# fverdoja/Fast-3D-Pointcloud-Segmentation

Hardware: AMD Instinct MI355X
Metric: Mpoints/sec segmented end-to-end, 1M-pt RGB-D frames (higher is better)
Workload: dtype f32

## Files before the change

### fast-3d-pointcloud-segmentation_amd/csrc/f3ds_algo.h

```cpp
#ifndef F3DS_ALGO_H_
#define F3DS_ALGO_H_

#include "f3ds_numerics.h"

namespace f3ds {

#define F3DS_MAX_SEED_EVENTS 48
struct SeedEvent {
    int trigger;
    int depth;
    double min[3];
    unsigned off[3];
};
struct SeedGrid {
    int n_events;
    int error;
    int defined;
    int depth;
    double res;
    double min[3], max[3];
    unsigned off[3];
    SeedEvent ev[F3DS_MAX_SEED_EVENTS];
};
F3DS_HD void a_seed_init(SeedGrid& g, float seed_res) {
// ... 398 lines not shown
    }
    *owner_out = o; *dist_out = d;
}
F3DS_HD void a_centroid_finish(const float sum[9], unsigned count, float row[12]) {
    float nx = sum[6], ny = sum[7], nz = sum[8];
    float z = (nx * nx + ny * ny) + (nz * nz + 0.0f);
    if (z > 0.0f) { float q = n_sqrtf(z); nx /= q; ny /= q; nz /= q; }
    float c = (float)count;
    row[0] = sum[0] / c; row[1] = sum[1] / c; row[2] = sum[2] / c;
    row[3] = sum[3] / c; row[4] = sum[4] / c; row[5] = sum[5] / c;
    row[6] = nx; row[7] = ny; row[8] = nz;
    row[9] = row[10] = row[11] = 0.0f;
}

F3DS_HD void a_payload_row(const float* vf_row, float out[12]) {
    float x = vf_row[0], y = vf_row[1], z = vf_row[2];
    out[0] = x * x; out[1] = x * y; out[2] = x * z; out[3] = y * y; out[4] = y * z; out[5] = z * z;
    out[6] = x; out[7] = y; out[8] = z;
    out[9] = (float)((uint32_t)vf_row[3] & 255u);
    out[10] = (float)((uint32_t)vf_row[4] & 255u);
    out[11] = (float)((uint32_t)vf_row[5] & 255u);
}
F3DS_HD void a_fold_row(float acc[12], const float row[12], unsigned index_plus_1) {
    for (int k = 0; k < 9; ++k) acc[k] += row[k];
    float count = (float)index_plus_1;
    float inv = 1 / count;
    for (int k = 9; k < 12; ++k) acc[k] = acc[k] + inv * (row[k] - acc[k]);
}
F3DS_HD void a_region_from_acc(const float acc[12], unsigned count, float rec[16]) {
    float c = (float)count;
    rec[0] = acc[6] / c; rec[1] = acc[7] / c; rec[2] = acc[8] / c;
    float n4[4];
    n_plane_normal(acc, count, rec, n4);
    rec[3] = n4[0]; rec[4] = n4[1]; rec[5] = n4[2];
    rec[6] = acc[9]; rec[7] = acc[10]; rec[8] = acc[11];
    n_rgb2lab(rec + 6, rec + 9);
    rec[12] = rec[13] = rec[14] = rec[15] = 0.0f;
}

struct MergeParams {
    int color_metric, geom_metric, merging;
    float lambda;
    int bins;
    const float* cdf_c;
    const float* cdf_g;
};
F3DS_HD float a_tc(const MergeParams& p, float dc, int* err) {
    if (p.merging != 2) return p.lambda * dc;
    short bin = (short)__builtin_floorf(dc * (float)(short)p.bins);
    if (bin == (short)p.bins) bin--;
    if (bin < 0 || bin >= (short)p.bins) { *err = -9; return 0.0f; }
    return p.cdf_c[bin] / 2;
}
F3DS_HD float a_tg(const MergeParams& p, float dg, int* err) {
    if (p.merging != 2) return (1 - p.lambda) * dg;
    short bin = (short)__builtin_floorf(dg * (float)(short)p.bins);
    if (bin < 0 || bin >= (short)p.bins) { *err = -9; return 0.0f; }
    return p.cdf_g[bin] / 2;
}
template <class K = m_lit> F3DS_HD float a_edge_weight(const MergeParams& p, const float* rec_first, const float* rec_second, int* err, K mc = K()) {
    float dc, dg;
    n_delta_c_g(rec_first, rec_second, p.color_metric, p.geom_metric, &dc, &dg, mc);
    return a_tc(p, dc, err) + a_tg(p, dg, err);
}

struct EdgeHist {
    const uint32_t* ev_epoch;
    const uint32_t* ev_key;
    const int* ev_prev;
};
F3DS_HD bool a_edge_before(const EdgeHist& H, uint32_t e, uint32_t ke, int he, uint32_t f, uint32_t kf, int hf) {
    if (ke != kf) return ke < kf;
    for (;;) {
        uint32_t te = H.ev_epoch[he], tf = H.ev_epoch[hf];
        uint32_t tau = te > tf ? te : tf;
        if (tau == 0u) return e < f;
        if (te == tau) he = H.ev_prev[he];
        if (tf == tau) hf = H.ev_prev[hf];
        ke = H.ev_key[he]; kf = H.ev_key[hf];
        if (ke != kf) return ke < kf;
    }
}

}
#endif
```

### fast-3d-pointcloud-segmentation_amd/csrc/f3ds_hip.hip

```cpp
#include <hip/hip_runtime.h>

#include <algorithm>
#include <cmath>
#include <atomic>
#include <map>
#include <chrono>
#include <cstdio>
#include <cstdlib>
#include <cstring>
#include <string>
#include <type_traits>
#include <mutex>
#include <set>
#include <vector>

#include "../../include/f3ds.h"
#include "f3ds_algo.h"
#include "f3ds_glasbey.h"
#include "f3ds_eval.h"
#include "f3ds_dev.h"
#include "f3ds_levels.h"

using namespace f3ds;

#include "f3ds_kernels.inc"
#include "f3ds_levels.inc"

namespace {

thread_local std::string g_last_hip_error;
#define HIPCHECK(expr) do { hipError_t e_ = (expr); if (e_ != hipSuccess) { g_last_hip_error = std::string(#expr) + ": " + hipGetErrorString(e_); return F3DS_ERR_HIP; } } while (0)

template <class... Ts> struct ArgPack;
template <> struct ArgPack<> {};
template <class T, class... Ts> struct ArgPack<T, Ts...> { T head; ArgPack<Ts...> tail; };

template <class K, class... Done>
__device__ __forceinline__ void unpack_call(const ArgPack<>&, Done... d) { K{}(d...); }
template <class K, class T, class... Ts, class... Done>
__device__ __forceinline__ void unpack_call(const ArgPack<T, Ts...>& p, Done... d) { unpack_call<K>(p.tail, d..., p.head); }

template <class K, class = void> struct waves_per_simd { static constexpr int v = 1; };
template <class K> struct waves_per_simd<K, std::void_t<decltype(K::WAVES_PER_SIMD)>> { static constexpr int v = K::WAVES_PER_SIMD; };
template <class K, class = void> struct is_latency_kernel { static constexpr bool v = false; };
template <class K> struct is_latency_kernel<K, std::void_t<decltype(K::LATENCY_KERNEL)>> { static constexpr bool v = K::LATENCY_KERNEL; };
template <class K, class Pack>
__global__ __launch_bounds__(K::BLOCK, waves_per_simd<K>::v) void k_batched(const Pack* frames) {
#ifndef F3DS_EXP_NO_LATENCY_PRIO
    if constexpr (is_latency_kernel<K>::v) __builtin_amdgcn_s_setprio(3);
#endif
    const Pack p = frames[f3ds_frame()];
    unpack_call<K>(p);
}

template <class F> struct op_traits;
template <class C, class... Ps> struct op_traits<void (C::*)(Ps...) const> { using pack = ArgPack<std::decay_t<Ps>...>; };
template <class K> using pack_of = typename op_traits<decltype(&K::operator())>::pack;

inline void fill_pack(ArgPack<>&) {}
template <class T, class... Ts, class A, class... As>
inline void fill_pack(ArgPack<T, Ts...>& p, A a, As... as) {
    static_assert(std::is_convertible<A, T>::value && !(std::is_pointer<T>::value && std::is_integral<A>::value),
                  "rec<K>(): an argument does not convert implicitly to the kernel's parameter type (wrong element type, swapped arguments?)");
    p.head = a; fill_pack(p.tail, as...);
}

typedef hipError_t (*LaunchFn)(uint32_t gx, uint32_t nf, uint32_t lds, hipStream_t st, const void* dargs);
template <class K>
hipError_t launch_fn(uint32_t gx, uint32_t nf, uint32_t lds, hipStream_t st, const void* dargs) {
    using Pack = pack_of<K>;
    if (lds > 48u * 1024u) {
        hipError_t e = hipFuncSetAttribute(reinterpret_cast<const void*>(k_batched<K, Pack>), hipFuncAttributeMaxDynamicSharedMemorySize, (int)lds);
        if (e != hipSuccess) return e;
    }
    hipLaunchKernelGGL((k_batched<K, Pack>), dim3(gx ? gx : 1u, nf), dim3(K::BLOCK), lds, st, static_cast<const Pack*>(dargs));
    return hipGetLastError();
}
struct Cmd { LaunchFn fn; uint32_t gx, lds, bytes, off; };

const int g_inc_shift = [] { const char* e = dev_getenv("F3DS_INC_SHIFT"); return e ? atoi(e) : 6; }();

struct Switches {
    bool direct_labels = false, copy_stream = true, copy_duplex = false, split_voxel_accum = false, sweep_tiles = true, merge_spec = true, force_global_merge = false, no_stream_pool = false, sort_pairs = false, host_prof = false, trace_err = false, vox_hash = true, vox_tiles_forced = false, levels_global = false;
    int normals_threads = 0, merge_nw = 0, merge_keys = -1; uint32_t tile_holes = 0, ilist_slack = 32, r_rounds = F3DS_R_ROUNDS; long relabel_lds_cap = -1;
    void read() {
        auto on = [](const char* n) { return dev_getenv(n) != nullptr; };
        auto num = [](const char* n, long dflt) { const char* e = dev_getenv(n); return e ? atol(e) : dflt; };
        direct_labels = num("F3DS_DIRECT_LABELS", 0) != 0; copy_stream = num("F3DS_COPY_STREAM", 1) != 0; copy_duplex = num("F3DS_COPY_STREAM", 1) == 2; split_voxel_accum = on("F3DS_SPLIT_VOXEL_ACCUM"); sweep_tiles = num("F3DS_SWEEP_TILES", 1) != 0; merge_spec = num("F3DS_MERGE_SPEC", 1) != 0;
        force_global_merge = on("F3DS_FORCE_GLOBAL_MERGE"); no_stream_pool = on("F3DS_NO_STREAM_POOL"); sort_pairs = on("F3DS_SORT_PAIRS");
        host_prof = on("F3DS_HOST_PROF"); trace_err = on("F3DS_TRACE_ERR");
        vox_tiles_forced = num("F3DS_VOX_TILES", 1) == 2;
        vox_hash = num("F3DS_VOX_TILES", 1) != 0 && !sort_pairs && !split_voxel_accum;
        normals_threads = (int)num("F3DS_NORMALS_THREADS", 0); tile_holes = (uint32_t)num("F3DS_SWEEP_TILE_HOLES", 0);
        { const long v = num("F3DS_MERGE_NW", 0); merge_nw = v == 4 ? 4 : (v ? 8 : 0); }
        { const char* e = dev_getenv("F3DS_MERGE_KEYS"); merge_keys = !e ? -1 : (!strcmp(e, "lds") ? 2 : (!strcmp(e, "global") ? 1 : 0)); }
        relabel_lds_cap = num("F3DS_RELABEL_LDS_CAP", -1);
        levels_global = num("F3DS_LEVELS_GLOBAL", 0) != 0;
        { const long v = num("F3DS_R_ROUNDS_RUN", F3DS_R_ROUNDS); r_rounds = v >= 1 && v <= F3DS_R_ROUNDS ? (uint32_t)v : (uint32_t)F3DS_R_ROUNDS; }
        { const long v = num("F3DS_ILIST_SLACK", 32); ilist_slack = v >= 1 && v <= 32 ? (uint32_t)v : 32u; }
    }
};
thread_local Switches g_sw;
const int g_merge_shared_res = [] { const char* e = dev_getenv("F3DS_MERGE_SHARED_RES"); return e && atoi(e) == 2 ? 2 : 0; }();

#define F3DS_SCRATCH(X) \
    X(P16, pts) X(P16, spts) X(uint64_t, keys0) X(uint64_t, keys1) X(uint32_t, vals0) X(uint32_t, vals1) X(uint32_t, flags) X(uint32_t, incl) X(uint32_t, tiles) X(uint32_t, hist) X(uint32_t, seg_start) X(int, pt_voxel) X(uint32_t, labels) \
    X(uint32_t, vkey) X(uint32_t, vcount) X(float, vf) X(int, nbr) X(int, nbrT) X(uint64_t, hkeys) X(uint32_t, hvals) X(float, boxes) X(uint32_t, ckey) X(uint32_t, cell_start) X(uint64_t, chk) X(uint32_t, chv) X(uint32_t, chvals) X(int, seed_orig) X(uint32_t, keep) X(int, seed_kept) \
    X(uint32_t, owner0) X(uint32_t, ownR) X(float, dist0) X(unsigned char, R) X(float, hc) X(uint32_t, hcount) X(uint32_t, hlo) X(uint32_t, hhi) X(int, ghost_vox) X(unsigned char, ghost_active) X(unsigned char, ghost_done) X(uint32_t, ghost_head) X(uint32_t, ghost_next) \
    X(uint32_t, loff) X(float, rows) X(int, row_voxel) X(float, racc0) X(uint32_t, rcnt0) X(float, rrec0) X(unsigned char, ralive0) X(uint64_t, ehk) X(uint64_t, ekeys0) X(uint64_t, ekeys1) X(uint32_t, evals0) X(uint32_t, evals1) X(uint32_t, ea0) X(uint32_t, eb0) \
    X(uint32_t, ea) X(uint32_t, eb) X(float, ew) X(uint32_t, eku) X(int, ehist) X(unsigned char, ealive) X(uint32_t, ev_epoch) X(uint32_t, ev_key) X(int, ev_prev) X(float, racc) X(uint32_t, rcnt) X(float, rrec) X(unsigned char, ralive) X(uint32_t, rhead) X(uint32_t, rtail) X(uint32_t, lnext) X(uint32_t, parent) X(uint32_t, markA) X(uint32_t, markB) X(uint32_t, tl) X(uint32_t, merges) \
     X(float, r_vf) X(uint32_t, r_owner) X(float, r_dist) X(float, r_hc) X(uint32_t, r_hcount) X(uint32_t, r_hlo) X(uint32_t, r_hhi) X(int, r_gvox) X(unsigned char, r_gact) X(unsigned char, r_gdone) X(uint32_t, r_ghead) X(uint32_t, r_gnext) X(uint32_t, r_tl) X(uint32_t, r_tcnt) X(int, r_seed) X(uint32_t, r_L) \
    X(uint32_t, tstamp) X(uint32_t, tround) X(uint32_t, hdirty) X(uint32_t, htiles) X(uint32_t, htcnt) X(uint32_t, vwl) X(uint32_t, vwl2) X(uint32_t, vtmask) \
     X(uint32_t, glut) X(uint32_t, truth_pts) X(uint32_t, tsum) X(uint32_t, tcol) X(uint32_t, tlab) X(uint32_t, ctab) X(uint32_t, csize) X(uint32_t, eroot) X(uint32_t, eincl) \
     X(uint32_t, hcnt) X(uint32_t, pslot) X(uint32_t, vlist) \
     X(uint32_t, u_src) X(uint32_t, u_voff) X(float, u_xyz) X(uint32_t, u_rgba) X(float, u_cent) X(float, u_nrm) \
    X(float, deltas) X(uint64_t, skeys0) X(uint64_t, skeys1) X(uint32_t, svals0) X(uint32_t, svals1) X(uint32_t, cdf_hist) X(float, cdf) X(uint32_t, root) X(uint32_t, rincl) X(uint32_t, rrank) X(uint2, pool) X(uint32_t, rstart) X(uint32_t, rnleaf) X(uint32_t, rcap) X(uint32_t, tile_n1) X(uint32_t, tile_ord) X(uint32_t, tile_slots) X(uint32_t, ilist) X(uint32_t, istart) X(uint32_t, ilen) X(uint32_t, icap) \
     X(uint32_t, lv_into) X(uint32_t, lv_at) X(uint32_t, lv_pfx) X(float, lv_thr) X(uint32_t, lv_tab) X(uint32_t, lv_nreg) X(uint32_t, lv_out)
template <class T> struct Scratch { T* p = nullptr; size_t cap = 0; int slot = -1; };
#define F3DS_SCRATCH_SLOT(T, name) S_##name,
#define F3DS_SCRATCH_MEMBER(T, name) Scratch<T> name{nullptr, 0, S_##name};
#define F3DS_SCRATCH_VISIT(T, name) if (const int rc_ = f(name)) return rc_;
enum ScratchSlot { F3DS_SCRATCH(F3DS_SCRATCH_SLOT) N_SCRATCH };

}

struct f3ds_ctx {
    int device = 0;
    hipStream_t own_stream = nullptr;
    hipStream_t stream = nullptr;
    hipEvent_t ev[11] = {};
    DevCounters* d_dc = nullptr;
    DevCounters* h_dc = nullptr;
    GridInfo* d_grid = nullptr;
    GridInfo* h_grid = nullptr;
    SeedGrid* d_sgrid = nullptr;
    std::vector<Cmd> cmds;
    std::vector<unsigned char> blob;
    std::vector<uintptr_t> pend;
    MultiOp ops = {}; uint32_t ops_grid = 0;
    unsigned char* h_args[2] = {nullptr, nullptr}; unsigned char* d_args[2] = {nullptr, nullptr}; size_t args_cap = 0;
    hipEvent_t ev_args[2] = {nullptr, nullptr}; bool args_used[2] = {false, false}; int args_flip = 0;
    hipEvent_t ev_copy[3] = {nullptr, nullptr, nullptr};
    DevCounters* d_dcblk = nullptr; DevCounters* h_dcblk = nullptr; size_t dcblk_cap = 0;
    bool have_frame = false;
    bool live = false;
    int rc = 0;
    f3ds_params prm;
    FrameArgs fa;
    const P16* d_pts = nullptr;
    uint32_t n = 0, V = 0, C = 0, S0 = 0, E = 0, hmask = 0;
    uint64_t *ks = nullptr; uint32_t *vs = nullptr;
    uint64_t *cks = nullptr; uint32_t *cvs = nullptr;
    uint64_t *eks = nullptr;
    f3ds_result res;
    bool merge_in_lds = false;
    int merge_kind = 0;
    uint32_t ev_mult = 64;
    uint32_t pool_mult = 1;
    uint32_t vox_cap = 0;
    bool vox_hashed = false;
    bool vox_dense = false;
    uint32_t vox_dense_wait = 0, vox_dense_penalty = 8;
    uint32_t ilist_mult = 1;
    uint32_t edge_mult = 32;
    bool relabel_lds = true;
    int refined_itr = -1;
    int idxbits = -1;
    uint32_t* user_labels = nullptr;
    MergeDev mdev; MergeLds mlds; float host_lambda = 0.5f;
    F3DS_SCRATCH(F3DS_SCRATCH_MEMBER)
    template <class F> int each_scratch(F&& f) { F3DS_SCRATCH(F3DS_SCRATCH_VISIT) return 0; }
    std::vector<uint32_t> tsize;
    float cluster_T = 0.0f;
    bool user_mode = false;
    std::vector<uint32_t> user_label, user_row;
};

namespace {

bool referenced_by_pending_calls(const f3ds_ctx* c, const void* mem, size_t cap) {
    const uintptr_t lo = (uintptr_t)mem, hi = lo + cap;
    for (const uintptr_t w : c->pend) if (w >= lo && w < hi) return true;
    for (uint32_t k = 0; k < c->ops.n; ++k) {
        const uintptr_t d = (uintptr_t)c->ops.dst[k], sp = (uintptr_t)c->ops.src[k];
        if ((d >= lo && d < hi) || (sp >= lo && sp < hi)) return true;
    }
    return false;
}
template <class A> inline void note_arg(f3ds_ctx* c, const A& a) {
    if constexpr (std::is_pointer<A>::value) { if (a) c->pend.push_back((uintptr_t)a); }
    else if constexpr (std::is_class<A>::value) {
        static_assert(std::is_trivially_copyable<A>::value, "kernel arguments must be plain data");
        for (size_t off = 0; off + 8 <= sizeof(A); off += 8) { uintptr_t w; memcpy(&w, reinterpret_cast<const unsigned char*>(&a) + off, 8); if (w) c->pend.push_back(w); }
    }
}
std::atomic<size_t> g_scratch_hwm[16][N_SCRATCH];
std::atomic<unsigned long long> g_scratch_allocs{0};
template <class T>
int regrow(Scratch<T>& b, size_t mark) {
    g_scratch_allocs.fetch_add(1, std::memory_order_relaxed);
    if (b.p) { HIPCHECK(hipFree(b.p)); b.p = nullptr; b.cap = 0; }
    const size_t want = mark + mark / 4 + 64;
    HIPCHECK(hipMalloc(&b.p, want));
    b.cap = want;
    return F3DS_OK;
}
template <class T>
int ensure(f3ds_ctx* c, Scratch<T>& b, size_t count, T** out) {
    size_t bytes = count * sizeof(T);
    if (bytes < 256) bytes = 256;
    size_t target = bytes;
    std::atomic<size_t>& hwm = g_scratch_hwm[c->device & 15][b.slot];
    size_t seen = hwm.load(std::memory_order_relaxed);
    while (seen < bytes && !hwm.compare_exchange_weak(seen, bytes, std::memory_order_relaxed)) {}
    if (seen > target && seen <= 4 * bytes) target = seen;
    if (b.cap < bytes) {
        if (b.p && (!c->cmds.empty() || c->ops.n) && referenced_by_pending_calls(c, b.p, b.cap)) {
            fprintf(stderr, "f3ds: internal error: regrowing a buffer that a recorded kernel call refers to\n");
            return F3DS_ERR_LOGIC;
        }
        static const bool trace = dev_getenv("F3DS_TRACE_ALLOC") != nullptr;
        if (trace && b.p) fprintf(stderr, "f3ds: regrow slot %d: cap %zu, request %zu, mark %zu, pending calls %zu\n", b.slot, b.cap, bytes, target, c->cmds.size());
        if (const int rc = regrow(b, target)) return rc;
    }
    *out = b.p;
    return F3DS_OK;
}
int pregrow_scratch(f3ds_ctx* c) {
    return c->each_scratch([c](auto& b) -> int {
        if (!b.p) return F3DS_OK;
        const size_t mark = g_scratch_hwm[c->device & 15][b.slot].load(std::memory_order_relaxed);
        if (b.cap >= mark || mark > 4 * b.cap) return F3DS_OK;
        return regrow(b, mark);
    });
}
#define ENSURE(buf, count, ptr) do { int rc_ = ensure(c, buf, (size_t)(count), &ptr); if (rc_) return rc_; } while (0)

thread_local size_t g_grid_cap = 2048;
thread_local int g_batch_frames = 1;
std::atomic<int> g_batch_calls[16];
struct BatchCallCount { int d; explicit BatchCallCount(int dev) : d(dev & 15) { g_batch_calls[d].fetch_add(1, std::memory_order_relaxed); } ~BatchCallCount() { g_batch_calls[d].fetch_sub(1, std::memory_order_relaxed); } };
size_t grid_cap_for_batch(int frames) {
    static const size_t target = dev_getenv("F3DS_GRID_TARGET") ? (size_t)atol(dev_getenv("F3DS_GRID_TARGET")) : 3072;
    if (!target) return 2048;
    size_t cap = target / (size_t)(frames > 0 ? frames : 1);
    return cap < 8 ? 8 : (cap > 2048 ? 2048 : cap);
}
inline uint32_t grid_wide(size_t work, int block) {
    size_t g = (work + block - 1) / block;
    return (uint32_t)(g < 1 ? 1 : (g > 2048 ? 2048 : g));
}
inline uint32_t grid_for(size_t work, int block) {
    size_t g = (work + block - 1) / block;
    if (g < 1) g = 1;
    if (g > g_grid_cap) g = g_grid_cap;
    return (uint32_t)g;
}
inline uint32_t pow2_ge(size_t x) { uint32_t p = 1; while (p < x) p <<= 1; return p; }
int bits_for(uint64_t max_value) { int b = 0; while (b < 64 && (max_value >> b)) ++b; return b; }

template <class K, class... As> void rec(f3ds_ctx* c, uint32_t gx, uint32_t lds, As... as);
inline void flush_ops(f3ds_ctx* c) {
    if (!c->ops.n) return;
    const MultiOp m = c->ops; const uint32_t g = c->ops_grid;
    c->ops.n = 0; c->ops_grid = 0;
    rec<d_multi_op>(c, g, 0u, m);
}
template <class K, class... As>
void rec(f3ds_ctx* c, uint32_t gx, uint32_t lds, As... as) {
    if constexpr (!std::is_same<K, d_multi_op>::value) flush_ops(c);
    using Pack = pack_of<K>;
    static_assert(std::is_trivially_copyable<Pack>::value, "kernel arguments must be plain data");
    Pack p;
    memset(&p, 0, sizeof p);
    fill_pack(p, as...);
    (note_arg(c, as), ...);
    Cmd cmd; cmd.fn = &launch_fn<K>; cmd.gx = gx; cmd.lds = lds; cmd.bytes = (uint32_t)sizeof(Pack); cmd.off = (uint32_t)c->blob.size();
    c->blob.resize(c->blob.size() + sizeof(Pack));
    memcpy(c->blob.data() + cmd.off, &p, sizeof(Pack));
    c->cmds.push_back(cmd);
}
inline void rec_op(f3ds_ctx* c, void* dst, const void* src, uint32_t value, size_t bytes) {
    const uint32_t words = (uint32_t)((bytes + 3) / 4);
    if (c->ops.n == (uint32_t)MULTI_OPS) flush_ops(c);
    MultiOp& m = c->ops;
    if (m.n == 0) memset(&m, 0, sizeof m);
    m.dst[m.n] = static_cast<uint32_t*>(dst); m.src[m.n] = static_cast<const uint32_t*>(src); m.val[m.n] = value; m.words[m.n] = words; m.n++;
    const uint32_t g = grid_for(words, 256);
    if (g > c->ops_grid) c->ops_grid = g;
}
inline void rec_fill(f3ds_ctx* c, void* dst, uint32_t value, size_t bytes) { rec_op(c, dst, nullptr, value, bytes); }
inline void rec_copy(f3ds_ctx* c, void* dst, const void* src, size_t bytes) { rec_op(c, dst, src, 0u, bytes); }
inline void reset_recording(f3ds_ctx* c) { c->cmds.clear(); c->blob.clear(); c->pend.clear(); c->ops.n = 0; c->ops_grid = 0; }

struct Batch {
    std::vector<f3ds_ctx*> fr;
    hipStream_t st = nullptr;
    f3ds_ctx* owner = nullptr;
};

thread_local double g_t_wait = 0, g_t_launch = 0;
static int trace_err(int code, const char* where, const f3ds_ctx* c) {
    if (code && g_sw.trace_err)
        fprintf(stderr, "f3ds: error %d after %s (V %u, seeds %u, edges %u, chain overflow %d, capacity flag %d)\n", code, where, c->V, c->S0, c->h_dc->n_edges,
                c->h_dc->r_overflow, c->h_dc->ev_overflow);
    return code;
}
static inline double now_ms() { return std::chrono::duration<double, std::milli>(std::chrono::steady_clock::now().time_since_epoch()).count(); }
inline hipError_t timed_sync(hipEvent_t e) { const double t0 = now_ms(); const hipError_t r = hipEventSynchronize(e); g_t_wait += now_ms() - t0; return r; }
inline hipError_t timed_sync(hipStream_t st) { const double t0 = now_ms(); const hipError_t r = hipStreamSynchronize(st); g_t_wait += now_ms() - t0; return r; }
template <class F> int clear_counter(f3ds_ctx* c, hipStream_t st, F DevCounters::*f) { c->h_dc->*f = 0; HIPCHECK(hipMemsetAsync(&(c->d_dc->*f), 0, sizeof(F), st)); return F3DS_OK; }
template <class... Fs> int clear_counters(f3ds_ctx* c, hipStream_t st, Fs DevCounters::*... f) { int rc = F3DS_OK; (void)((rc = clear_counter(c, st, f)) || ...); return rc; }
int flush(Batch& b, hipEvent_t before_launch = nullptr) {
    if (b.fr.empty()) return F3DS_OK;
    for (f3ds_ctx* c : b.fr) flush_ops(c);
    const size_t ncmd = b.fr[0]->cmds.size();
    for (f3ds_ctx* c : b.fr) if (c->cmds.size() != ncmd) return F3DS_ERR_UNSUPPORTED;
    if (ncmd == 0) return F3DS_OK;
    const uint32_t nf = (uint32_t)b.fr.size();
    size_t total = 0;
    std::vector<size_t> off(ncmd);
    for (size_t j = 0; j < ncmd; ++j) { off[j] = total; total += (((size_t)b.fr[0]->cmds[j].bytes * nf) + 63u) & ~(size_t)63u; }
    f3ds_ctx* o = b.owner;
    if (o->args_cap < total) {
        HIPCHECK(hipStreamSynchronize(b.st));
        for (int k = 0; k < 2; ++k) {
            if (o->h_args[k]) HIPCHECK(hipHostFree(o->h_args[k]));
            if (o->d_args[k]) HIPCHECK(hipFree(o->d_args[k]));
            o->h_args[k] = o->d_args[k] = nullptr; o->args_used[k] = false;
        }
        o->args_cap = total * 2;
        for (int k = 0; k < 2; ++k) {
            HIPCHECK(hipHostMalloc(&o->h_args[k], o->args_cap, hipHostMallocDefault));
            HIPCHECK(hipMalloc(&o->d_args[k], o->args_cap));
            if (!o->ev_args[k]) HIPCHECK(hipEventCreateWithFlags(&o->ev_args[k], hipEventDisableTiming));
        }
    }
    const int fl = o->args_flip; o->args_flip ^= 1;
    if (o->args_used[fl]) HIPCHECK(timed_sync(o->ev_args[fl]));
    unsigned char* const h_args = o->h_args[fl]; unsigned char* const d_args = o->d_args[fl];
    const double tl0 = now_ms();
    for (size_t j = 0; j < ncmd; ++j)
        for (uint32_t i = 0; i < nf; ++i) {
            const Cmd& cm = b.fr[i]->cmds[j];
            if (cm.fn != b.fr[0]->cmds[j].fn) return F3DS_ERR_UNSUPPORTED;
            memcpy(h_args + off[j] + (size_t)i * cm.bytes, b.fr[i]->blob.data() + cm.off, cm.bytes);
        }
    HIPCHECK(hipMemcpyAsync(d_args, h_args, total, hipMemcpyHostToDevice, b.st));
    if (before_launch) HIPCHECK(hipEventRecord(before_launch, b.st));
    for (size_t j = 0; j < ncmd; ++j) {
        uint32_t gx = 1, lds = 0;
        for (uint32_t i = 0; i < nf; ++i) { const Cmd& cm = b.fr[i]->cmds[j]; if (cm.gx > gx) gx = cm.gx; if (cm.lds > lds) lds = cm.lds; }
        HIPCHECK(b.fr[0]->cmds[j].fn(gx, nf, lds, b.st, d_args + off[j]));
    }
    HIPCHECK(hipEventRecord(o->ev_args[fl], b.st)); o->args_used[fl] = true;
    for (f3ds_ctx* c : b.fr) reset_recording(c);
    g_t_launch += now_ms() - tl0;
    return F3DS_OK;
}
int flush_sync(Batch& b) {
    int rc = flush(b);
    if (rc) return rc;
    const size_t nf = b.fr.size();
    if (nf == 1) HIPCHECK(hipMemcpyAsync(b.fr[0]->h_dc, b.fr[0]->d_dc, sizeof(DevCounters), hipMemcpyDeviceToHost, b.st));
    else if (nf > 1) {
        f3ds_ctx* o = b.owner;
        if (o->dcblk_cap < nf) {
            HIPCHECK(hipStreamSynchronize(b.st));
            if (o->d_dcblk) HIPCHECK(hipFree(o->d_dcblk));
            if (o->h_dcblk) HIPCHECK(hipHostFree(o->h_dcblk));
            o->dcblk_cap = nf * 2;
            HIPCHECK(hipMalloc(&o->d_dcblk, o->dcblk_cap * sizeof(DevCounters)));
            HIPCHECK(hipHostMalloc(&o->h_dcblk, o->dcblk_cap * sizeof(DevCounters), hipHostMallocDefault));
        }
        for (size_t i = 0; i < nf; ++i) rec<d_dc_gather>(b.fr[i], 1u, 0u, b.fr[i]->d_dc, o->d_dcblk + i);
        if ((rc = flush(b))) return rc;
        HIPCHECK(hipMemcpyAsync(o->h_dcblk, o->d_dcblk, nf * sizeof(DevCounters), hipMemcpyDeviceToHost, b.st));
    }
    HIPCHECK(timed_sync(b.st));
    HIPCHECK(hipGetLastError());
    if (nf > 1) for (size_t i = 0; i < nf; ++i) *b.fr[i]->h_dc = b.owner->h_dcblk[i];
// ... 207 lines not shown
    if (sb.reseed) {
        rec<d_reseed_own>(c, grid_for(S0, 256), 0u, sb.seeds, S0, owner0);
        rec<d_reseed_init>(c, grid_for(S0 + 1, 256), 0u, sb.seeds, S0, owner0, ghost_vox, ghost_active, ghost_done, hlo, hhi, hcount, tl, tcnt);
    } else {
        rec<d_helper_own>(c, grid_for(S0, 256), 0u, sb.seeds, S0, owner0);
        rec<d_helper_init>(c, grid_for(S0 + 1, 256), 0u, sb.seeds, S0, owner0, ghost_vox, ghost_active, ghost_done, hlo, hhi, hcount, hc, tl, tcnt);
    }
    const int* nbrT = c->nbrT.p; const float* vf = sb.vf;
    SweepFrame a;
    a.sv = SweepView{(int)V, nbrT, vf, owner0, dist0, hc, ghost_head, ghost_next, &c->d_dc->n_ghosts, prm.seed_res, prm.w_normal, prm.w_color, prm.w_spatial, c->nbr.p};
    a.R = R; a.ownR = ownR; a.owner_out = owner0; a.dist_out = dist0;
    a.ghost_done = ghost_done; a.ghost_active = ghost_active; a.ghost_vox = ghost_vox; a.ghost_head = ghost_head; a.ghost_next = ghost_next;
    a.hlo = hlo; a.hhi = hhi; a.hcount = hcount; a.hc = hc; a.dc = c->d_dc; a.S0 = S0;
    a.tR0 = tiles4; a.tR1 = tiles4 + T; a.tC0 = tiles4 + 2 * (size_t)T; a.tC1 = tiles4 + 3 * (size_t)T; a.tRr = trr; a.hD = hD; a.T = T; a.tl = tl; a.tcnt = tcnt; a.wl = wl; a.wl2 = wl2; a.tmask = tmask;
    a.thr = g_inc_shift >= 32 ? 0xFFFFFFFFu : (g_inc_shift < 0 ? 0u : V >> g_inc_shift);
    if (!g_sw.sweep_tiles) a.tile_n1 = nullptr;
    else a.tile_n1 = c->tile_n1.p;
    a.tile_ord = c->tile_ord.p; a.tile_slots = c->tile_slots.p;
    for (uint32_t t = 0; t < c->res.sweeps; ++t) {
        if (a_sweep_needs_clear(t)) rec_fill(c, R, 0u, V);
        rec<d_sweep_begin>(c, 1u, 0u, a, t);
        const bool can_skip = t >= 2u;
        const bool rounds = g_inc_shift >= 0 && can_skip;
        const uint32_t nrounds = rounds ? g_sw.r_rounds : 0u;
        rec<d_sweep_R_first>(c, grid_for(V, 256), 0u, a, a_sweep_tag(t), t, nrounds);
        for (uint32_t r = 1; r < nrounds; ++r) rec<d_sweep_R_round>(c, grid_for(V, 256), 0u, a, t, r, nrounds);
        for (uint32_t pass = 0; pass < F3DS_R_PASSES; ++pass) rec<d_sweep_R>(c, pass == 0 ? grid_for(V, 256) : 64u, 0u, a, a_sweep_tag(t), t, pass);
        rec<d_sweep_R_tail>(c, 1u, 0u, a, a_sweep_tag(t), t);
        rec<d_sweep_claim>(c, grid_for(V, 256), 0u, a, t);
        rec<d_centroid>(c, grid_for((size_t)S0 * 64u, 256), 0u, a, t);
    }
    return F3DS_OK;
}
int seg_sweeps(f3ds_ctx* c) {
    SweepBufs sb{&c->owner0, &c->dist0, &c->hc, &c->hcount, &c->hlo, &c->hhi, &c->ghost_vox, &c->ghost_active, &c->ghost_done, &c->ghost_head, &c->ghost_next, &c->htiles, &c->htcnt, c->vf.p, c->seed_kept.p, false};
    return seg_sweeps_on(c, sb);
}
int seg_supervoxels(f3ds_ctx* c) {
    const uint32_t V = c->V, S0 = c->S0;
    uint32_t *loff, *rcnt0, *ev0, *ev1; float *rows, *racc0, *rrec0; int* row_voxel; unsigned char* ralive0; uint64_t *ehk, *ek0, *ek1;
    ENSURE(c->loff, S0 + 2, loff);
    int rc = scan_u32(c, c->hcount.p, loff + 1, S0 + 1);
    if (rc) return rc;
    rec_fill(c, loff, 0u, 4);
    ENSURE(c->rows, ((size_t)V + S0 + 1) * 12, rows); ENSURE(c->row_voxel, (size_t)V + S0 + 1, row_voxel);
    ENSURE(c->racc0, (size_t)(S0 + 1) * 12, racc0); ENSURE(c->rcnt0, S0 + 1, rcnt0); ENSURE(c->rrec0, (size_t)(S0 + 1) * 16, rrec0);
    ENSURE(c->ralive0, S0 + 1, ralive0);
    rec_fill(c, ralive0, 0u, S0 + 1);
    rec_fill(c, rcnt0, 0u, (size_t)(S0 + 1) * 4);
    rec<d_sv_fill>(c, S0 ? (S0 + 3u) / 4u : 1u, 0u,
                   c->vf.p, c->owner0.p, S0, c->hlo.p, c->hhi.p, c->ghost_vox.p, c->ghost_active.p, c->hcount.p, loff, c->hc.p, rows, row_voxel, racc0, rcnt0, rrec0, ralive0, c->d_dc, c->htiles.p, c->htcnt.p, V);
    const uint32_t ecap = (uint32_t)std::min<uint64_t>((uint64_t)S0 * c->edge_mult + 1024u, 0x7fffffffu);
    const uint32_t ehcap = pow2_ge((size_t)ecap * 2);
    ENSURE(c->ehk, ehcap, ehk);
    ENSURE(c->ekeys0, ecap, ek0); ENSURE(c->ekeys1, ecap, ek1); ENSURE(c->evals0, ecap, ev0); ENSURE(c->evals1, ecap, ev1);
    rec_fill(c, ehk, 0xFFFFFFFFu, (size_t)ehcap * 8);
    rec<d_edges>(c, grid_for(V, 256), 0u, V, S0, c->nbrT.p, c->owner0.p, ehk, ehcap - 1, ek0, ecap, c->d_dc);
    rec<d_edges_ghost>(c, grid_for(S0, 256), 0u, V, S0, c->ghost_vox.p, c->ghost_active.p, c->nbrT.p, c->owner0.p, ehk, ehcap - 1, ek0, ecap, c->d_dc);
    return F3DS_OK;
}
int seg_edge_sort(f3ds_ctx* c, int sort_bits) {
    const uint32_t E = c->E, S0 = c->S0;
    uint32_t *ea0, *eb0; ENSURE(c->ea0, E, ea0); ENSURE(c->eb0, E, eb0);
    uint32_t* evs;
    { uint32_t* h; ENSURE(c->hist, (size_t)RS_BINS * (((size_t)E * 2 + RS_TILE - 1) / RS_TILE + 1), h); }
    rec<d_iota>(c, grid_for(E, 256), 0u, c->evals0.p, E);
    int rc = radix_sort(c, c->ekeys0.p, c->evals0.p, c->ekeys1.p, c->evals1.p, E, sort_bits, &c->eks, &evs);
    if (rc) return rc;
    rec<d_edge_init>(c, grid_for(E, 256), 0u, c->eks, E, S0, ea0, eb0);
    return F3DS_OK;
}
bool merge_il_layout(uint32_t E, uint32_t S0, int nw, int res, MergeLds* xl) {
    memset(xl, 0, sizeof *xl);
    if ((uint64_t)E * (res == 2 ? 10u : 2u) > (1u << 22)) return false;
    const MergeIlLayout L = merge_il_offsets(E, nw, res);
    xl->Ecap = L.Ecap; xl->NGcap = L.NGcap; xl->lds_bytes = L.total; xl->keys_in_lds = res;
    xl->spec = g_sw.merge_spec ? 1 : 0;
    return L.total <= MC_LDS_LIMIT && S0 <= 65534u;
}
enum MergeKind { MK_GLOBAL = 0, MK_IL = 1 };
inline int mk_waves(int kind) { return (kind - MK_IL) >= 2 ? 4 : 8; }
inline int mk_res(int kind) { return (kind - MK_IL) % 2 ? 0 : 2; }
int choose_merge_kind(const std::vector<f3ds_ctx*>& fr, bool force_global) {
    if (force_global || g_sw.force_global_merge) return MK_GLOBAL;
    const bool e_keys = g_sw.merge_keys >= 0;
    const bool shared = fr.size() >= 16 && g_batch_calls[fr[0]->device & 15].load(std::memory_order_relaxed) >= 2;
    const int nw = g_sw.merge_nw ? (g_sw.merge_nw == 8 ? 8 : 4) : (shared ? 4 : 8);
    const int first = e_keys ? (g_sw.merge_keys == 2 ? 2 : 0) : (shared ? g_merge_shared_res : 2);
    for (int res = first; res >= (e_keys ? first : 0); res -= 2) {
        bool ok = true;
        for (f3ds_ctx* c : fr) { MergeLds t; if (!merge_il_layout(c->E, c->S0, nw, res, &t)) { ok = false; break; } }
        if (ok) return MK_IL + (nw == 8 ? 0 : 2) + (res == 2 ? 0 : 1);
    }
    return MK_GLOBAL;
}
int seg_cluster_front(f3ds_ctx* c, const f3ds_params* prm, int kind) {
    const bool use_lds = kind != MK_GLOBAL;
    const uint32_t S0 = c->S0, E = c->E;
    float lambda = 0.5f; int bins = 500;
    if (prm->merging == F3DS_MANUAL_LAMBDA && prm->lambda != 0) { if (prm->lambda < 0 || prm->lambda > 1) return F3DS_ERR_RANGE; lambda = prm->lambda; }
    if (prm->merging == F3DS_EQUALIZATION && prm->bins != 0) { if (prm->bins < 0) return F3DS_ERR_RANGE; bins = (short)prm->bins; }
    if (prm->merging < 0 || prm->merging > 2 || prm->color_metric < 0 || prm->color_metric > 1 || prm->geom_metric < 0 || prm->geom_metric > 1) return F3DS_ERR_ARG;
    MergeDev m;
    memset(&m, 0, sizeof m);
    m.E = E; m.S0 = S0; m.threshold = prm->threshold; m.dc = c->d_dc;
    { const uint64_t cap = (uint64_t)E * c->ev_mult + 4096u; m.ev_cap = cap > 0x7fffffffull ? 0x7fffffffu : (uint32_t)cap; }
    ENSURE(c->ea, E, m.ea); ENSURE(c->eb, E, m.eb); ENSURE(c->ew, ((size_t)E + 2047) & ~(size_t)2047, m.ew);  ENSURE(c->eku, ((size_t)E + 2047) & ~(size_t)2047, m.eku);
    ENSURE(c->ehist, E, m.ehist); ENSURE(c->ealive, E, m.ealive);
    ENSURE(c->ev_epoch, m.ev_cap, m.ev_epoch); ENSURE(c->ev_key, m.ev_cap, m.ev_key); ENSURE(c->ev_prev, m.ev_cap, m.ev_prev);
    ENSURE(c->racc, (size_t)(S0 + 1) * 12, m.racc); ENSURE(c->rrec, (size_t)(S0 + 1) * 16, m.rrec);
    ENSURE(c->rcnt, S0 + 1, m.rcnt); ENSURE(c->ralive, S0 + 1, m.ralive);
    ENSURE(c->rhead, S0 + 1, m.rhead); ENSURE(c->rtail, S0 + 1, m.rtail); ENSURE(c->lnext, S0 + 1, m.lnext);
    ENSURE(c->parent, S0 + 1, m.parent); ENSURE(c->markA, S0 + 1, m.markA); ENSURE(c->markB, S0 + 1, m.markB);
    ENSURE(c->tl, E, m.tl); ENSURE(c->merges, (size_t)(S0 + 1) * 3, m.merges);
    m.loff = c->loff.p; m.llen = c->hcount.p; m.rows = c->rows.p;
    float* deltas; ENSURE(c->deltas, (size_t)E * 2, deltas);
    rec_copy(c, m.racc, c->racc0.p, (size_t)(S0 + 1) * 12 * 4);
    rec_copy(c, m.rrec, c->rrec0.p, (size_t)(S0 + 1) * 16 * 4);
    rec_copy(c, m.rcnt, c->rcnt0.p, (size_t)(S0 + 1) * 4);
    rec_copy(c, m.ralive, c->ralive0.p, (size_t)(S0 + 1));
    rec_copy(c, m.ea, c->ea0.p, (size_t)E * 4);
    rec_copy(c, m.eb, c->eb0.p, (size_t)E * 4);
    MergeLds xl;
    merge_il_layout(E, S0, use_lds ? mk_waves(kind) : 8, use_lds ? mk_res(kind) : 0, &xl);
    uint32_t logS = 1; while ((1u << logS) < S0 + 2u) ++logS;
    xl.pool_cap = (S0 + 1u) * (4u * logS + 8u) * c->pool_mult;
    ENSURE(c->pool, xl.pool_cap, xl.pool); ENSURE(c->rstart, S0 + 1, xl.rstart); ENSURE(c->rnleaf, S0 + 1, xl.rnleaf);
    ENSURE(c->rcap, S0 + 1, xl.rcap);
    if (use_lds) {
        const uint64_t bound = 2ull * E + (uint64_t)(S0 ? S0 - 1u : 0u) * (MC_TL_CAP + MC_TL_CAP / 2u + 4u) + 1024u;
        uint64_t cap = 2ull * E + (uint64_t)g_sw.ilist_slack * E * c->ilist_mult + (g_sw.ilist_slack < 32u ? 16u : 1024u);
        if (cap > bound) cap = bound;
        xl.ilist_cap = cap > 0x7fffffffull ? 0x7fffffffu : (uint32_t)cap;
        ENSURE(c->ilist, xl.ilist_cap, xl.ilist); ENSURE(c->istart, S0 + 1, xl.istart); ENSURE(c->ilen, S0 + 1, xl.ilen); ENSURE(c->icap, S0 + 1, xl.icap);
    }
    if (use_lds) rec<d_inc_build>(c, 1u, 0u, E, S0, m.ea, m.eb, xl.istart, xl.ilen, xl.icap, xl.ilist);
    xl.stop_key = (prm->threshold != prm->threshold) ? 0u : n_weight_key(prm->threshold);
    c->merge_in_lds = use_lds; c->merge_kind = kind;
    rec<d_region_reset>(c, grid_for(S0 + 1, 256), 0u, S0, c->hcount.p, m.rhead, m.rtail, m.lnext, m.parent, m.markA, m.markB, xl.pool, xl.rstart, xl.rnleaf, xl.rcap, c->loff.p);
    m.mp.color_metric = prm->color_metric; m.mp.geom_metric = prm->geom_metric; m.mp.merging = prm->merging; m.mp.lambda = lambda; m.mp.bins = bins;
    uint64_t *sk0 = nullptr, *sk1 = nullptr; uint32_t *sv0 = nullptr, *sv1 = nullptr;
    if (prm->merging == F3DS_ADAPTIVE_LAMBDA) {
        ENSURE(c->skeys0, (size_t)E * 2, sk0); ENSURE(c->skeys1, (size_t)E * 2, sk1);
        ENSURE(c->svals0, (size_t)E * 2, sv0); ENSURE(c->svals1, (size_t)E * 2, sv1);
    }
    rec<d_edge_deltas>(c, grid_for(E, 256), 0u, E, m.ea, m.eb, m.rrec, prm->color_metric, prm->geom_metric, deltas, sk0, sv0);
    if (prm->merging == F3DS_ADAPTIVE_LAMBDA) {
        uint64_t* ks; uint32_t* vs;
        int rc = radix_sort(c, sk0, sv0, sk1, sv1, E * 2u, 33, &ks, &vs);
        if (rc) return rc;
        rec<d_lambda>(c, 1u, 0u, E, deltas, vs, c->d_dc);
    } else if (prm->merging == F3DS_EQUALIZATION) {
        uint32_t* hist; float* cdf;
        ENSURE(c->cdf_hist, (size_t)2 * (bins > 0 ? bins : 1), hist); ENSURE(c->cdf, (size_t)2 * (bins > 0 ? bins : 1), cdf);
        rec_fill(c, hist, 0u, (size_t)2 * (bins > 0 ? bins : 1) * 4);
        rec<d_cdf_hist>(c, grid_for((size_t)E * 2, 256), 0u, E, deltas, bins, hist, c->d_dc);
        rec<d_cdf_scan>(c, 1u, 0u, E, bins, hist, cdf);
        m.mp.cdf_c = cdf; m.mp.cdf_g = cdf + bins;
    }
    rec<d_edge_weights>(c, grid_for(E, 256), 0u, m, deltas);
    c->mdev = m; c->mlds = xl; c->host_lambda = lambda;
    return F3DS_OK;
}
int seg_merge(f3ds_ctx* c) {
#ifdef F3DS_WHATIF
    if (const char* e = dev_getenv("F3DS_FAKE_MERGE")) {
        unsigned us = 30000, waves = 1; sscanf(e, "%u,%u", &us, &waves);
        const char* l = dev_getenv("F3DS_FAKE_MERGE_LDS");
        rec<d_fake_merge>(c, 1u, l ? (uint32_t)atoi(l) * 1024u : c->mlds.lds_bytes, c->mdev, (uint32_t)us, (uint32_t)waves);
        return F3DS_OK;
    }
#endif
    switch (c->merge_kind) {
        case MK_IL + 0: rec<d_merge_il_t<8, 2>>(c, 1u, c->mlds.lds_bytes, c->mdev, c->mlds); break;
        case MK_IL + 1: rec<d_merge_il_t<8, 0>>(c, 1u, c->mlds.lds_bytes, c->mdev, c->mlds); break;
        case MK_IL + 2: rec<d_merge_il_t<4, 2>>(c, 1u, c->mlds.lds_bytes, c->mdev, c->mlds); break;
        case MK_IL + 3: rec<d_merge_il_t<4, 0>>(c, 1u, c->mlds.lds_bytes, c->mdev, c->mlds); break;
        default: rec<d_merge>(c, 1u, 0u, c->mdev);
    }
    return F3DS_OK;
}
int seg_labels(f3ds_ctx* c) {
    const uint32_t S0 = c->S0, n = c->n;
    const MergeDev& m = c->mdev;
    uint32_t *root, *rincl, *d_labels;
    ENSURE(c->root, S0 + 1, root); ENSURE(c->rincl, S0 + 1, rincl);
    if (c->user_labels) d_labels = c->user_labels;
    else ENSURE(c->labels, n, d_labels);
    if (c->relabel_lds) {
        const uint32_t gx = std::min(grid_for(n, 256), grid_wide(n, 4096));
        rec<d_relabel>(c, gx, (S0 + 1u) * 4u, n, c->pt_voxel.p, c->owner0.p, S0, m.parent, m.ralive, root, rincl, d_labels, c->d_dc);
    } else {
        uint32_t* rank; ENSURE(c->rrank, S0 + 1, rank);
        rec<d_region_ids>(c, 1u, 0u, S0, m.parent, m.ralive, rank, root, rincl, c->d_dc);
        rec<d_point_labels>(c, grid_for(n, 256), 0u, n, c->pt_voxel.p, c->owner0.p, rank, d_labels);
    }
    return F3DS_OK;
}

int finish_empty(f3ds_ctx* c, hipStream_t st, uint32_t* point_labels, int labels_on_device) {
    uint32_t* d_labels;
    ENSURE(c->labels, c->n ? c->n : 1, d_labels);
    if (c->n) {
        HIPCHECK(hipMemsetAsync(d_labels, 0xFF, (size_t)c->n * 4, st));
        if (point_labels) HIPCHECK(hipMemcpyAsync(point_labels, d_labels, (size_t)c->n * 4, labels_on_device ? hipMemcpyDefault : hipMemcpyDeviceToHost, st));
    }
    c->have_frame = false; c->live = false;
    return F3DS_OK;
}

struct CopyStream { std::mutex m; hipStream_t s = nullptr; };
CopyStream g_copy_stream[16][2];
hipStream_t copy_stream_of(int device, int which = 0) {
    CopyStream& c = g_copy_stream[device & 15][which & 1];
    std::lock_guard<std::mutex> lk(c.m);
    if (!c.s && hipStreamCreateWithFlags(&c.s, hipStreamNonBlocking) != hipSuccess) c.s = nullptr;
    return c.s;
}
struct BatchStreamPool { std::mutex m; hipStream_t s[8] = {}; bool busy[8] = {}; };
const int g_batch_stream_count = [] { const char* e = getenv("GPU_MAX_HW_QUEUES"); int n = e ? atoi(e) : 4; return n < 1 ? 1 : (n > 8 ? 8 : n); }();
BatchStreamPool g_batch_streams[16];
struct BatchStreamLease {
    int dev = -1, slot = -1;
    hipStream_t acquire(int device) {
        BatchStreamPool& p = g_batch_streams[device & 15];
        std::lock_guard<std::mutex> lk(p.m);
        if (!p.s[0]) for (int i = 0; i < g_batch_stream_count; ++i) if (hipStreamCreateWithFlags(&p.s[i], hipStreamNonBlocking) != hipSuccess) { p.s[i] = nullptr; return nullptr; }
        for (int i = 0; i < g_batch_stream_count; ++i) if (!p.busy[i] && p.s[i]) { p.busy[i] = true; dev = device & 15; slot = i; return p.s[i]; }
        return nullptr;
    }
    ~BatchStreamLease() { if (slot >= 0) { std::lock_guard<std::mutex> lk(g_batch_streams[dev].m); g_batch_streams[dev].busy[slot] = false; } }
};

template <class F>
int for_frames(Batch& b, F&& fn) {
    for (f3ds_ctx* c : b.fr) { int rc = fn(c); if (rc) return rc; }
    return F3DS_OK;
}
void stage_mark(Batch& b, int i) { (void)hipEventRecord(b.owner->ev[i], b.st); }

static uint32_t* pinned_device_alias(uint32_t* host) {
    hipPointerAttribute_t at;
    memset(&at, 0, sizeof at);
    if (hipPointerGetAttributes(&at, host) != hipSuccess) { (void)hipGetLastError(); return nullptr; }
    if (at.type != hipMemoryTypeHost || !at.devicePointer) return nullptr;
    return static_cast<uint32_t*>(at.devicePointer);
}

int run_cluster(Batch& b, const f3ds_params* prm, uint32_t* const* labels_of, const std::vector<int>& index_of, int labels_on_device, bool force_global = false) {
    const int kind = choose_merge_kind(b.fr, force_global);
    const bool all_lds = kind != MK_GLOBAL;
    int rc = for_frames(b, [&](f3ds_ctx* c) { return seg_cluster_front(c, prm, kind); });
    if (rc || (rc = flush(b))) return rc;
    stage_mark(b, 5);
    if ((rc = for_frames(b, seg_merge)) || (rc = flush(b))) return rc;
    stage_mark(b, 6);
    for (size_t i = 0; i < b.fr.size(); ++i) {
        uint32_t* out = labels_of ? labels_of[index_of[i]] : nullptr;
        if (out && !labels_on_device && g_sw.direct_labels) out = pinned_device_alias(out);
        else if (!labels_on_device) out = nullptr;
        b.fr[i]->user_labels = out;
    }
    {
        const uint32_t cap = g_sw.relabel_lds_cap >= 0 ? (uint32_t)g_sw.relabel_lds_cap : RL_LDS_CAP;
        bool fits = true;
        for (f3ds_ctx* c : b.fr) if (c->S0 + 1u > cap) fits = false;
        for (f3ds_ctx* c : b.fr) c->relabel_lds = fits;
    }
    if ((rc = for_frames(b, seg_labels)) || (rc = flush(b))) return rc;
    stage_mark(b, 7);
    {
        bool want = false;
        for (size_t i = 0; i < b.fr.size(); ++i) if (labels_of && labels_of[index_of[i]] && !b.fr[i]->user_labels && b.fr[i]->n) want = true;
        hipStream_t dl = (want && !labels_on_device && g_sw.copy_stream) ? copy_stream_of(b.fr[0]->device, g_sw.copy_duplex ? 1 : 0) : nullptr;
        if (dl) {
            for (int k = 1; k < 3; ++k) if (!b.owner->ev_copy[k]) HIPCHECK(hipEventCreateWithFlags(&b.owner->ev_copy[k], hipEventDisableTiming));
            HIPCHECK(hipEventRecord(b.owner->ev_copy[1], b.st));
            HIPCHECK(timed_sync(b.owner->ev_copy[1]));
        }
        for (size_t i = 0; i < b.fr.size(); ++i) {
            f3ds_ctx* c = b.fr[i];
            uint32_t* out = labels_of ? labels_of[index_of[i]] : nullptr;
            if (out && !c->user_labels && c->n) HIPCHECK(hipMemcpyAsync(out, c->labels.p, (size_t)c->n * 4, hipMemcpyDeviceToHost, dl ? dl : b.st));
            c->user_labels = nullptr;
        }
        if (dl) HIPCHECK(hipEventRecord(b.owner->ev_copy[2], dl));
        if ((rc = flush_sync(b))) return rc;
        if (dl) HIPCHECK(timed_sync(b.owner->ev_copy[2]));
    }
    {
        bool again = false;
        for (f3ds_ctx* c : b.fr) {
            if (c->h_dc->ev_overflow == 1 && c->ev_mult < 16384u) { c->ev_mult *= 4u; again = true; }
            if (c->h_dc->ev_overflow == 2 && c->pool_mult < 64u) { c->pool_mult *= 4u; again = true; }
            if (c->h_dc->ev_overflow == 4 && c->ilist_mult < 4096u) { c->ilist_mult *= 4u; again = true; }
        }
        if (again) {
            if (g_sw.trace_err) fprintf(stderr, "f3ds: merge stage of %zu frames runs again with more history / leaf-pool room\n", b.fr.size());
            for (f3ds_ctx* c : b.fr) if ((rc = clear_counters(c, b.st, &DevCounters::error, &DevCounters::ev_overflow))) return rc;
            return run_cluster(b, prm, labels_of, index_of, labels_on_device, force_global);
        }
    }
    if (all_lds) {
        bool again = false;
        for (f3ds_ctx* c : b.fr) if (c->h_dc->error == F3DS_ERR_UNSUPPORTED) again = true;
        if (again) {
            if (g_sw.trace_err) fprintf(stderr, "f3ds: merge stage of %zu frames runs again with the global-memory kernel\n", b.fr.size());
            for (f3ds_ctx* c : b.fr) if ((rc = clear_counters(c, b.st, &DevCounters::error))) return rc;
            return run_cluster(b, prm, labels_of, index_of, labels_on_device, true);
        }
    }
    for (f3ds_ctx* c : b.fr) {
        if (c->h_dc->error) return trace_err(c->h_dc->error, "merge", c);
        c->res.n_merges = c->h_dc->n_merges; c->res.n_regions = c->h_dc->n_regions;
        c->res.lambda = prm->merging == F3DS_ADAPTIVE_LAMBDA ? (c->E ? c->h_dc->lambda : __builtin_nanf("")) : c->host_lambda;
        c->prm.color_metric = prm->color_metric; c->prm.geom_metric = prm->geom_metric; c->prm.merging = prm->merging;
        c->prm.lambda = prm->lambda; c->prm.bins = prm->bins; c->prm.threshold = prm->threshold;
        c->cluster_T = prm->threshold;
        c->have_frame = true;
    }
    return F3DS_OK;
}

}

extern "C" {

const char* f3ds_last_hip_error(void) { return g_last_hip_error.c_str(); }

int f3ds_device_count(void) {
    int n = 0;
    if (hipGetDeviceCount(&n) != hipSuccess) return 0;
    return n;
}

int f3ds_create(int device, f3ds_ctx** out) {
    if (!out) return F3DS_ERR_ARG;
    *out = nullptr;
    int n = 0;
    if (hipGetDeviceCount(&n) != hipSuccess || n <= 0) return F3DS_ERR_NO_DEVICE;
    if (device < 0 || device >= n) return F3DS_ERR_ARG;
    HIPCHECK(hipSetDevice(device));
    f3ds_ctx* c = new f3ds_ctx;
    c->device = device;
    if (const char* e = dev_getenv("F3DS_EDGE_MULT")) { const int v = atoi(e); if (v >= 1 && v <= 32) c->edge_mult = (uint32_t)v; }
    const int rc = [c]() -> int {
        HIPCHECK(hipStreamCreateWithFlags(&c->own_stream, hipStreamNonBlocking));
        c->stream = c->own_stream;
        for (auto& e : c->ev) HIPCHECK(hipEventCreate(&e));
        HIPCHECK(hipMalloc(&c->d_dc, sizeof(DevCounters)));
        HIPCHECK(hipHostMalloc(&c->h_dc, sizeof(DevCounters), hipHostMallocDefault));
        HIPCHECK(hipMalloc(&c->d_grid, sizeof(GridInfo)));
        HIPCHECK(hipHostMalloc(&c->h_grid, sizeof(GridInfo), hipHostMallocDefault));
        HIPCHECK(hipMalloc(&c->d_sgrid, sizeof(SeedGrid)));
        return F3DS_OK;
    }();
    if (rc) { c->stream = c->own_stream; f3ds_destroy(c); return rc; }
    memset(c->h_grid, 0, sizeof(GridInfo));
    memset(&c->res, 0, sizeof c->res);
    *out = c;
    return F3DS_OK;
}

void f3ds_destroy(f3ds_ctx* c) {
    if (!c) return;
    (void)hipSetDevice(c->device);
    if (c->stream) (void)hipStreamSynchronize(c->stream);
    c->each_scratch([](auto& b) { if (b.p) (void)hipFree(b.p); return 0; });
    if (c->d_dc) (void)hipFree(c->d_dc);
    if (c->h_dc) (void)hipHostFree(c->h_dc);
    if (c->d_grid) (void)hipFree(c->d_grid);
    if (c->h_grid) (void)hipHostFree(c->h_grid);
    if (c->d_sgrid) (void)hipFree(c->d_sgrid);
    for (int k = 0; k < 2; ++k) { if (c->h_args[k]) (void)hipHostFree(c->h_args[k]); if (c->d_args[k]) (void)hipFree(c->d_args[k]); if (c->ev_args[k]) (void)hipEventDestroy(c->ev_args[k]); }
    for (auto& e : c->ev_copy) if (e) (void)hipEventDestroy(e);
    if (c->d_dcblk) (void)hipFree(c->d_dcblk);
    if (c->h_dcblk) (void)hipHostFree(c->h_dcblk);
    for (auto& e : c->ev) if (e) (void)hipEventDestroy(e);
    if (c->own_stream) (void)hipStreamDestroy(c->own_stream);
    delete c;
}

int f3ds_set_stream(f3ds_ctx* c, void* hip_stream) {
    if (!c) return F3DS_ERR_ARG;
    c->stream = hip_stream ? (hipStream_t)hip_stream : c->own_stream;
    return F3DS_OK;
}

int f3ds_segment(f3ds_ctx* c, const void* points, size_t n_, int points_on_device, const f3ds_params* prm, uint32_t* point_labels,
                 int labels_on_device, f3ds_result* result) {
    const void* pp[1] = {points}; const size_t cnt[1] = {n_}; uint32_t* lp[1] = {point_labels};
    return f3ds_segment_batch(&c, 1, pp, cnt, points_on_device, prm, lp, labels_on_device, result);
}

int f3ds_segment_batch(f3ds_ctx** ctxs, int nctx, const void* const* points, const size_t* counts, int points_on_device, const f3ds_params* prm,
                       uint32_t* const* point_labels, int labels_on_device, f3ds_result* results) {
    if (!ctxs || nctx <= 0 || !points || !counts || !prm) return F3DS_ERR_ARG;
    if (!(prm->voxel_res > 0) || !(prm->seed_res > 0)) return F3DS_ERR_ARG;
    for (int i = 0; i < nctx; ++i) if (!ctxs[i] || (!points[i] && counts[i]) || counts[i] > 0x7fffffffull || ctxs[i]->device != ctxs[0]->device) return F3DS_ERR_ARG;
    const auto t0 = std::chrono::steady_clock::now();
    g_t_wait = 0; g_t_launch = 0;
    g_sw.read();
    HIPCHECK(hipSetDevice(ctxs[0]->device));
    BatchCallCount in_flight(ctxs[0]->device);
    Batch b;
    b.owner = ctxs[0]; b.st = ctxs[0]->stream;
    BatchStreamLease lease;
    if (nctx > 1 && ctxs[0]->stream == ctxs[0]->own_stream && !g_sw.no_stream_pool) { hipStream_t ps = lease.acquire(ctxs[0]->device); if (ps) b.st = ps; }
    g_grid_cap = grid_cap_for_batch(nctx); g_batch_frames = nctx;
    std::vector<int> index_of;
    const int max_depth = (int)(1.8f * prm->seed_res / prm->voxel_res);
    const uint32_t sweeps = max_depth > 1 ? (uint32_t)(max_depth - 1) : 0u;
    stage_mark(b, 0);
    hipStream_t up_stream = (!points_on_device && g_sw.copy_stream) ? copy_stream_of(ctxs[0]->device) : nullptr;
    bool uploaded = false;
    for (int i = 0; i < nctx; ++i) {
        f3ds_ctx* c = ctxs[i];
        reset_recording(c);
        c->have_frame = false; c->live = true; c->rc = 0; c->refined_itr = -1;
        c->user_mode = false; c->user_label.clear(); c->user_row.clear();
        { const int prc = pregrow_scratch(c); if (prc) return prc; }
        c->prm = *prm; c->n = (uint32_t)counts[i]; c->V = c->C = c->S0 = c->E = 0;
        memset(&c->res, 0, sizeof c->res);
        c->res.n_points = c->n; c->res.sweeps = sweeps;
        c->fa = FrameArgs{prm->use_transform, prm->fold_negative_z, prm->leaf_order, prm->voxel_res, prm->seed_res, prm->w_color, prm->w_spatial, prm->w_normal};
        if (points_on_device) c->d_pts = static_cast<const P16*>(points[i]);
        else {
            P16* up; ENSURE(c->pts, c->n ? c->n : 1, up);
            if (c->n) { HIPCHECK(hipMemcpyAsync(up, points[i], (size_t)c->n * 16, hipMemcpyHostToDevice, up_stream ? up_stream : b.st)); uploaded = true; }
            c->d_pts = up;
        }
        b.fr.push_back(c); index_of.push_back(i);
    }
    if (up_stream && uploaded) {
        if (!b.owner->ev_copy[0]) HIPCHECK(hipEventCreateWithFlags(&b.owner->ev_copy[0], hipEventDisableTiming));
        HIPCHECK(hipEventRecord(b.owner->ev_copy[0], up_stream));
        HIPCHECK(hipStreamWaitEvent(b.st, b.owner->ev_copy[0], 0));
    }
    auto drop_dead = [&](auto&& dead) -> int {
        std::vector<f3ds_ctx*> keep; std::vector<int> keep_idx;
        for (size_t i = 0; i < b.fr.size(); ++i) {
            f3ds_ctx* c = b.fr[i];
            if (dead(c)) { int rc = finish_empty(c, b.st, point_labels ? point_labels[index_of[i]] : nullptr, labels_on_device); if (rc) return rc; }
            else { keep.push_back(c); keep_idx.push_back(index_of[i]); }
        }
        b.fr.swap(keep); index_of.swap(keep_idx);
        return F3DS_OK;
    };
    int rc;
    if ((rc = for_frames(b, seg_bbox)) || (rc = flush_sync(b))) return rc;
    for (f3ds_ctx* c : b.fr) {
        c->res.n_finite = c->h_dc->n_finite;
        if (c->h_dc->error) return c->h_dc->error;
        c->res.octree_depth = (uint32_t)c->h_dc->depth;
    }
    if ((rc = drop_dead([](f3ds_ctx* c) { return c->h_dc->grid_empty || c->n == 0; }))) return rc;
    int maxd = 0;
    for (f3ds_ctx* c : b.fr) if (c->h_dc->depth > maxd) maxd = c->h_dc->depth;
    bool hashed = g_sw.vox_hash && (nctx >= 4 || g_sw.vox_tiles_forced);
    for (f3ds_ctx* c : b.fr) {
        c->vox_hashed = false;
        if (c->vox_dense && hashed) { if (c->vox_dense_wait) c->vox_dense_wait--; else c->vox_dense = false; }
    }
    for (f3ds_ctx* c : b.fr) if (c->vox_dense) hashed = false;
    if (hashed) {
        uint32_t maxtiles = 1;
        for (f3ds_ctx* c : b.fr) maxtiles = std::max(maxtiles, (c->n + VT_TILE - 1u) / VT_TILE);
        const int tile_bits = bits_for((uint64_t)maxtiles - 1u);
        rc = for_frames(b, [&](f3ds_ctx* c) { return seg_vox_tiles(c, 3 * maxd, tile_bits); });
        if (rc == F3DS_ERR_UNSUPPORTED) {
            for (f3ds_ctx* c : b.fr) { reset_recording(c); c->vox_hashed = false; }
            hashed = false;
        } else if (rc || (rc = flush_sync(b))) return rc;
        if (hashed && g_sw.trace_err) for (f3ds_ctx* c : b.fr) fprintf(stderr, "f3ds: tile path: most voxels in a tile %u, descriptors %u, leaves %u, lists sorted %u\n", c->h_dc->vox_max_tile, c->h_dc->seg_count, c->h_dc->n_voxels, c->h_dc->vox_disorder);
        if (hashed) for (f3ds_ctx* c : b.fr) if (c->h_dc->ev_overflow == 6 || c->h_dc->ev_overflow == 7) {
            if (g_sw.trace_err) fprintf(stderr, "f3ds: tile path refused a frame: %s (descriptors %u, leaves %u)\n", c->h_dc->ev_overflow == 6 ? "a voxel with too many points" : "a tile with too many voxels", c->h_dc->seg_count, c->h_dc->n_voxels);
            c->vox_dense = true; c->vox_dense_wait = c->vox_dense_penalty; c->vox_dense_penalty = std::min(2u * c->vox_dense_penalty, 1024u); hashed = false;
        }
        if (!hashed) {
            if (g_sw.trace_err) fprintf(stderr, "f3ds: voxelisation of %zu frames runs again on the sort path (an unorganised cloud or dense voxels)\n", b.fr.size());
            for (f3ds_ctx* c : b.fr) {
                c->vox_hashed = false;
                if ((rc = clear_counters(c, b.st, &DevCounters::error, &DevCounters::ev_overflow, &DevCounters::n_voxels, &DevCounters::seg_count))) return rc;
            }
        }
    }
    if (!hashed) {
        uint32_t maxn = 1;
        for (f3ds_ctx* c : b.fr) if (c->n > maxn) maxn = c->n;
// ... 109 lines not shown
                const auto it = std::lower_bound(lab.begin() + 1, lab.end(), l);
                if (it == lab.end() || *it != l) return F3DS_ERR_OUT_OF_RANGE;
                hh[w] = (uint32_t)(it - lab.begin());
            }
            if (hh[0] == hh[1] || !seen.insert({hh[0], hh[1]}).second) return F3DS_ERR_ARG;
            ed.push_back({hh[0], hh[1]});
        }
        std::stable_sort(ed.begin(), ed.end(), [](const std::pair<uint32_t, uint32_t>& a, const std::pair<uint32_t, uint32_t>& b) { return a.first < b.first; });
        if (ed.size() > 0x7fffffffull) return F3DS_ERR_UNSUPPORTED;
        ea.resize(ed.size()); eb.resize(ed.size());
        for (size_t k = 0; k < ed.size(); ++k) { ea[k] = ed[k].first; eb[k] = ed[k].second; }
    }
    const uint32_t E = (uint32_t)ea.size();
    reset_recording(c);
    c->have_frame = false; c->live = true; c->rc = 0; c->refined_itr = -1;
    { const int prc = pregrow_scratch(c); if (prc) return prc; }
    c->prm = *prm; c->n = Vt; c->V = c->C = 0; c->S0 = S; c->E = E; c->d_pts = nullptr;
    memset(&c->res, 0, sizeof c->res);
    c->res.n_voxels = Vt; c->res.n_seeds = S; c->res.n_supervoxels = S; c->res.n_edges = E;
    c->user_mode = true; c->user_label = lab; c->user_row = row;
    if (S == 0) {
        c->user_mode = false; c->user_label.clear(); c->user_row.clear(); c->live = false;
        if (result) *result = c->res;
        return F3DS_OK;
    }
    Batch b; b.owner = c; b.st = c->stream; b.fr.push_back(c); g_grid_cap = grid_cap_for_batch(1); g_batch_frames = 1;
    uint32_t *d_src, *d_voff, *d_rgba, *loff, *hcount, *owner, *rcnt0, *ea0, *eb0; float *d_xyz, *d_cent, *d_nrm, *rows, *racc0, *rrec0, *hc; int *row_voxel, *pt_voxel; unsigned char* ralive0;
    ENSURE(c->u_src, S + 1u, d_src); ENSURE(c->u_voff, S + 1u, d_voff); ENSURE(c->u_xyz, (size_t)Vt * 3, d_xyz); ENSURE(c->u_rgba, Vt, d_rgba);
    ENSURE(c->u_cent, (size_t)S * 3, d_cent); ENSURE(c->u_nrm, (size_t)S * 3, d_nrm);
    ENSURE(c->loff, S + 2u, loff); ENSURE(c->hcount, S + 1u, hcount); ENSURE(c->owner0, Vt, owner); ENSURE(c->pt_voxel, Vt, pt_voxel);
    ENSURE(c->rows, ((size_t)Vt + S + 1) * 12, rows); ENSURE(c->row_voxel, (size_t)Vt + S + 1, row_voxel);
    ENSURE(c->racc0, (size_t)(S + 1) * 12, racc0); ENSURE(c->rcnt0, S + 1u, rcnt0); ENSURE(c->rrec0, (size_t)(S + 1) * 16, rrec0);
    ENSURE(c->ralive0, S + 1u, ralive0); ENSURE(c->hc, (size_t)(S + 1) * 12, hc);
    ENSURE(c->ea0, E, ea0); ENSURE(c->eb0, E, eb0);
    std::vector<uint32_t> h_loff(S + 2u, 0u), h_cnt(S + 1u, 0u);
    for (uint32_t h = 1; h <= S; ++h) { h_loff[h] = sv->voxel_offset[row[h]]; h_cnt[h] = sv->voxel_offset[row[h] + 1] - sv->voxel_offset[row[h]]; }
    h_loff[S + 1] = Vt;
    const hipStream_t st = b.st;
    HIPCHECK(hipMemcpyAsync(d_src, row.data(), (size_t)(S + 1) * 4, hipMemcpyHostToDevice, st));
    HIPCHECK(hipMemcpyAsync(d_voff, sv->voxel_offset, (size_t)(S + 1) * 4, hipMemcpyHostToDevice, st));
    HIPCHECK(hipMemcpyAsync(d_xyz, sv->voxel_xyz, (size_t)Vt * 12, hipMemcpyHostToDevice, st));
    HIPCHECK(hipMemcpyAsync(d_rgba, sv->voxel_rgba, (size_t)Vt * 4, hipMemcpyHostToDevice, st));
    HIPCHECK(hipMemcpyAsync(d_cent, sv->centroid_xyz, (size_t)S * 12, hipMemcpyHostToDevice, st));
    HIPCHECK(hipMemcpyAsync(d_nrm, sv->normal, (size_t)S * 12, hipMemcpyHostToDevice, st));
    HIPCHECK(hipMemcpyAsync(loff, h_loff.data(), (size_t)(S + 2) * 4, hipMemcpyHostToDevice, st));
    HIPCHECK(hipMemcpyAsync(hcount, h_cnt.data(), (size_t)(S + 1) * 4, hipMemcpyHostToDevice, st));
    if (E) { HIPCHECK(hipMemcpyAsync(ea0, ea.data(), (size_t)E * 4, hipMemcpyHostToDevice, st)); HIPCHECK(hipMemcpyAsync(eb0, eb.data(), (size_t)E * 4, hipMemcpyHostToDevice, st)); }
    stage_mark(b, 4);
    rec<d_init_counters>(c, 1u, 0u, c->d_dc);
    rec_fill(c, ralive0, 0u, S + 1u);
    rec_fill(c, rcnt0, 0u, (size_t)(S + 1) * 4);
    rec_fill(c, racc0, 0u, 48); rec_fill(c, rrec0, 0u, 64); rec_fill(c, hc, 0u, 48);
    rec<d_iota>(c, grid_for(Vt, 256), 0u, reinterpret_cast<uint32_t*>(pt_voxel), Vt);
    rec<d_sv_user_fill>(c, S, 0u, S, d_src, d_voff, d_xyz, d_rgba, d_cent, d_nrm, rows, row_voxel, owner, racc0, rcnt0, rrec0, ralive0, hc, c->d_dc);
    int rc = flush(b);
    if (rc) return rc;
    uint32_t* lp[1] = {voxel_labels}; std::vector<int> idx{0};
    if ((rc = run_cluster(b, prm, lp, idx, 0))) return rc;
    HIPCHECK(hipStreamSynchronize(b.st));
    for (int k = 4; k < 7; ++k) { float ms = 0; if (hipEventElapsedTime(&ms, c->ev[k], c->ev[k + 1]) == hipSuccess) c->res.ms_stage[k] = ms; }
    if (region_of_sv) {
        std::vector<uint32_t> root(S + 1u);
        HIPCHECK(hipMemcpy(root.data(), c->root.p, (size_t)(S + 1) * 4, hipMemcpyDeviceToHost));
        for (uint32_t i = 0; i < S; ++i) region_of_sv[i] = lab[root[hof[i]]];
    }
    c->live = false;
    c->res.ms_total = (float)std::chrono::duration<double, std::milli>(std::chrono::steady_clock::now() - t0).count();
    if (result) *result = c->res;
    return F3DS_OK;
}

}

namespace {
template <class T>
int fetch(f3ds_ctx* c, const Scratch<T>& b, size_t count, std::vector<T>& out) {
    out.resize(count);
    if (count) HIPCHECK(hipMemcpy(out.data(), b.p, count * sizeof(T), hipMemcpyDeviceToHost));
    return F3DS_OK;
}
inline uint32_t label_out(const f3ds_ctx* c, uint32_t h) { return c->user_mode && h < c->user_label.size() ? c->user_label[h] : h; }
int region_leaves(f3ds_ctx* c, std::vector<unsigned char>& ralive, std::vector<std::vector<uint2>>& leaves) {
    const uint32_t S0 = c->S0;
    std::vector<uint32_t> rhead, lnext, loff, llen, rstart, rnleaf; std::vector<uint2> pool;
    int rc;
    if ((rc = fetch(c, c->ralive, S0 + 1, ralive)) || (rc = fetch(c, c->rhead, S0 + 1, rhead)) || (rc = fetch(c, c->lnext, S0 + 1, lnext)) ||
        (rc = fetch(c, c->loff, S0 + 2, loff)) || (rc = fetch(c, c->hcount, S0 + 1, llen)))
        return rc;
    if (c->merge_in_lds && ((rc = fetch(c, c->pool, c->pool.cap / 8, pool)) || (rc = fetch(c, c->rstart, S0 + 1, rstart)) || (rc = fetch(c, c->rnleaf, S0 + 1, rnleaf)))) return rc;
    leaves.assign(S0 + 1, {});
    for (uint32_t h = 1; h <= S0; ++h) {
        if (!ralive[h]) continue;
        if (c->merge_in_lds) leaves[h].assign(pool.begin() + rstart[h], pool.begin() + rstart[h] + rnleaf[h]);
        else for (uint32_t leaf = rhead[h]; leaf; leaf = lnext[leaf]) leaves[h].push_back(make_uint2(loff[leaf], llen[leaf]));
    }
    return F3DS_OK;
}
inline size_t rows_in_use(const f3ds_ctx* c, const std::vector<uint32_t>& loff) { return c->user_mode ? c->n : loff[c->S0 + 1]; }
}

extern "C" int f3ds_get_regions(f3ds_ctx* c, uint32_t* label, uint32_t* n_voxels, float* centroid_xyz, float* normal, float* mean_rgb, size_t cap, size_t* n_out) {
    if (!c) return F3DS_ERR_ARG;
    if (!c->have_frame) return F3DS_ERR_LOGIC;
    HIPCHECK(hipSetDevice(c->device));
    HIPCHECK(hipStreamSynchronize(c->stream));
    const uint32_t S0 = c->S0;
    std::vector<unsigned char> ralive; std::vector<uint32_t> rcnt; std::vector<float> rrec;
    int rc;
    if ((rc = fetch(c, c->ralive, S0 + 1, ralive)) || (rc = fetch(c, c->rcnt, S0 + 1, rcnt)) || (rc = fetch(c, c->rrec, (size_t)(S0 + 1) * 16, rrec))) return rc;
    size_t k = 0;
    for (uint32_t h = 1; h <= S0; ++h) {
        if (!ralive[h]) continue;
        if (k < cap) {
            const float* r = &rrec[(size_t)h * 16];
            if (label) label[k] = label_out(c, h);
            if (n_voxels) n_voxels[k] = rcnt[h];
            if (centroid_xyz) { centroid_xyz[3 * k] = r[0]; centroid_xyz[3 * k + 1] = r[1]; centroid_xyz[3 * k + 2] = r[2]; }
            if (normal) { normal[3 * k] = r[3]; normal[3 * k + 1] = r[4]; normal[3 * k + 2] = r[5]; }
            if (mean_rgb) { mean_rgb[3 * k] = r[6]; mean_rgb[3 * k + 1] = r[7]; mean_rgb[3 * k + 2] = r[8]; }
        }
        k++;
    }
    if (n_out) *n_out = k;
    return (k > cap && (label || n_voxels || centroid_xyz || normal || mean_rgb)) ? F3DS_ERR_CAPACITY : F3DS_OK;
}

extern "C" int f3ds_get_region_voxels(f3ds_ctx* c, float* xyz, uint32_t* rgba, uint32_t* voxel_index, size_t cap, size_t* n_out) {
    if (!c) return F3DS_ERR_ARG;
    if (!c->have_frame) return F3DS_ERR_LOGIC;
    HIPCHECK(hipSetDevice(c->device));
    HIPCHECK(hipStreamSynchronize(c->stream));
    std::vector<unsigned char> ralive; std::vector<std::vector<uint2>> leaves; std::vector<float> rows; std::vector<int> rv; std::vector<uint32_t> loff;
    int rc;
    if ((rc = region_leaves(c, ralive, leaves)) || (rc = fetch(c, c->loff, c->S0 + 2, loff))) return rc;
    const size_t nrows = rows_in_use(c, loff);
    if ((rc = fetch(c, c->rows, nrows * 12, rows)) || (rc = fetch(c, c->row_voxel, nrows, rv))) return rc;
    size_t k = 0;
    for (uint32_t h = 1; h <= c->S0; ++h)
        for (const uint2& leaf : leaves[h])
            for (uint32_t j = 0; j < leaf.y; ++j) {
                if (k < cap) {
                    const float* r = &rows[(size_t)(leaf.x + j) * 12];
                    if (xyz) { xyz[3 * k] = r[6]; xyz[3 * k + 1] = r[7]; xyz[3 * k + 2] = r[8]; }
                    if (rgba) rgba[k] = (uint32_t)r[9] << 16 | (uint32_t)r[10] << 8 | (uint32_t)r[11];
                    if (voxel_index) voxel_index[k] = (uint32_t)rv[leaf.x + j];
                }
                k++;
            }
    if (n_out) *n_out = k;
    return (k > cap && (xyz || rgba || voxel_index)) ? F3DS_ERR_CAPACITY : F3DS_OK;
}

extern "C" int f3ds_get_voxel_cloud(f3ds_ctx* c, float* xyz, uint32_t* label, uint32_t* rgba, size_t cap, size_t* n_out) {
    if (!c) return F3DS_ERR_ARG;
    if (!c->have_frame) return F3DS_ERR_LOGIC;
    HIPCHECK(hipSetDevice(c->device));
    HIPCHECK(hipStreamSynchronize(c->stream));
    const uint32_t S0 = c->S0;
    std::vector<unsigned char> ralive; std::vector<std::vector<uint2>> all_leaves; std::vector<uint32_t> loff; std::vector<float> rows;
    int rc;
    if ((rc = region_leaves(c, ralive, all_leaves)) || (rc = fetch(c, c->loff, S0 + 2, loff))) return rc;
    if ((rc = fetch(c, c->rows, rows_in_use(c, loff) * 12, rows))) return rc;
    size_t k = 0; uint32_t cur = 0;
    for (uint32_t h = 1; h <= S0; ++h) {
        if (!ralive[h]) continue;
        const std::vector<uint2>& leaves = all_leaves[h];
        for (const uint2& leaf : leaves)
            for (uint32_t j = 0; j < leaf.y; ++j) {
                if (k < cap) {
                    const float* r = &rows[(size_t)(leaf.x + j) * 12];
                    if (xyz) { xyz[3 * k] = r[6]; xyz[3 * k + 1] = r[7]; xyz[3 * k + 2] = r[8]; }
                    if (label) label[k] = cur;
                    if (rgba) rgba[k] = f3ds_glasbey_256[cur % 256u];
                }
                k++;
            }
// ... 473 lines not shown
```

### fast-3d-pointcloud-segmentation_amd/csrc/f3ds_kernels.inc

```


namespace {

struct P16 { float x, y, z; uint32_t rgba; };

struct DevCounters {
    unsigned long long n_finite;
    uint32_t bbox[6];
    uint32_t bbox_any;
    uint32_t n_valid;
    uint32_t n_voxels;
    uint32_t n_cells;
    uint32_t n_seeds;
    uint32_t n_edges;
    uint32_t n_alive;
    uint32_t n_merges;
    uint32_t n_regions;
    uint32_t n_events;
    int error;
    int r_overflow;
    float lambda;
    uint32_t seg_count;
    uint32_t n_ghosts;
    int depth;
// ... 2705 lines not shown
    }
};
struct d_lambda {
    static constexpr bool LATENCY_KERNEL = true;
    static constexpr int BLOCK = 64;
    __device__ void operator()(uint32_t E, const float* deltas, const uint32_t* svals, DevCounters* dc) const {
        const int lane = lane_id();
        float count = 0, mean_d = 0;
        for (uint32_t base = 0; base < E; base += 64u) {
            const uint32_t i = base + lane;
            const float vc = i < E ? deltas[svals[i]] : 0.0f;
            const float vg = i < E ? deltas[svals[(size_t)E + i]] : 0.0f;
            const int nb = E - base < 64u ? (int)(E - base) : 64;
            const float inv = 1 / (count + (float)(lane + 1));
    #pragma unroll
            for (int j = 0; j < 64; ++j) {
                if (j < nb) {
                    const float dcj = __builtin_bit_cast(float, __builtin_amdgcn_readlane(__builtin_bit_cast(int, vc), j));
                    const float dgj = __builtin_bit_cast(float, __builtin_amdgcn_readlane(__builtin_bit_cast(int, vg), j));
                    const float ij = __builtin_bit_cast(float, __builtin_amdgcn_readlane(__builtin_bit_cast(int, inv), j));
                    const float d = lane == 0 ? dcj : dgj;
                    mean_d = mean_d + ij * (d - mean_d);
                }
            }
            count += (float)nb;
        }
        const float mean_c = __shfl(mean_d, 0, 64), mean_g = __shfl(mean_d, 1, 64);
        if (lane == 0) dc->lambda = mean_g / (mean_c + mean_g);
    }
};
struct d_cdf_hist {
    static constexpr int BLOCK = 256;
    __device__ void operator()(uint32_t E, const float* deltas, int bins, uint32_t* hist, DevCounters* dc) const {
        for (uint32_t t = BIX * blockDim.x + threadIdx.x; t < 2u * E; t += gridDim.x * blockDim.x) {
            const uint32_t w = t / E, e = t - w * E;
            const float d = deltas[e * 2 + w];
            short bin = (short)__builtin_floorf(d * (float)(short)bins);
            if (bin == (short)bins) bin--;
            if (bin < 0 || bin >= (short)bins) { dc->error = F3DS_ERR_EQ_BIN; continue; }
            atomicAdd(&hist[w * (uint32_t)bins + (uint32_t)bin], 1u);
        }
    }
};
struct d_cdf_scan {
    static constexpr bool LATENCY_KERNEL = true;
    static constexpr int BLOCK = 64;
    __device__ void operator()(uint32_t E, int bins, const uint32_t* hist, float* cdf) const {
        const int w = threadIdx.x;
        if (w >= 2) return;
        float v = 0;
        for (int i = 0; i < bins; ++i) { v += (float)hist[w * bins + i]; cdf[w * bins + i] = v / (float)(int)E; }
    }
};
struct MergeDev {
    uint32_t E, S0;
    uint32_t *ea, *eb; float* ew; uint32_t* eku; int* ehist; unsigned char* ealive;
    uint32_t *ev_epoch, *ev_key; int* ev_prev; uint32_t ev_cap;
    float *racc, *rrec; uint32_t* rcnt; unsigned char* ralive;
    uint32_t *rhead, *rtail, *lnext, *parent;
    const uint32_t *loff, *llen; const float* rows;
    uint32_t *markA, *markB, *tl;
    uint32_t* merges;
    float threshold;
    MergeParams mp;
    DevCounters* dc;
};
struct d_edge_weights {
    static constexpr int BLOCK = 256;
    __device__ void operator()(MergeDev m, const float* deltas) const {
        MergeParams mp = m.mp;
        if (mp.merging == 1) mp.lambda = m.dc->lambda;
        for (uint32_t e = BIX * blockDim.x + threadIdx.x; e < m.E; e += gridDim.x * blockDim.x) {
            int err = 0;
            const float w = a_tc(mp, deltas[e * 2], &err) + a_tg(mp, deltas[e * 2 + 1], &err);
            if (err) m.dc->error = err;
            m.ew[e] = w; m.eku[e] = n_weight_key(w); m.ehist[e] = (int)e; m.ealive[e] = 1;
            m.ev_epoch[e] = 0u; m.ev_key[e] = m.eku[e]; m.ev_prev[e] = -1;
        }
    }
};
struct d_region_reset {
    static constexpr int BLOCK = 256;
    __device__ void operator()(uint32_t S0, const uint32_t* hcount, uint32_t* rhead, uint32_t* rtail, uint32_t* lnext, uint32_t* parent,
                                                     uint32_t* markA, uint32_t* markB, uint2* pool, uint32_t* rstart, uint32_t* rnleaf, uint32_t* rcap,
                                                     const uint32_t* loff) const {
        for (uint32_t h = BIX * blockDim.x + threadIdx.x; h <= S0; h += gridDim.x * blockDim.x) {
            const bool alive = h > 0 && hcount[h] > 0;
            rhead[h] = alive ? h : 0u; rtail[h] = alive ? h : 0u; lnext[h] = 0u; parent[h] = h; markA[h] = 0u; markB[h] = 0u;
            pool[h] = make_uint2(loff[h], hcount[h]); rstart[h] = h; rnleaf[h] = alive ? 1u : 0u; rcap[h] = 1u;
        }
    }
};

constexpr int MG_THREADS = 1024;
__device__ inline bool edge_before(const MergeDev& m, uint32_t e, uint32_t f) {
    EdgeHist H{m.ev_epoch, m.ev_key, m.ev_prev};
    return a_edge_before(H, e, m.eku[e], m.ehist[e], f, m.eku[f], m.ehist[f]);
}
struct d_merge {
    static constexpr int BLOCK = MG_THREADS;
    __device__ void operator()(MergeDev m) const {
        __shared__ int s_wbest[MG_THREADS / 64];
        __shared__ uint32_t s_a, s_b, s_ntouched, s_nmerges, s_nevents;
        __shared__ int s_stop;
        const int tid = threadIdx.x, lane = lane_id(), wave = tid >> 6;
        MergeParams mp = m.mp;
        if (mp.merging == 1) mp.lambda = m.dc->lambda;
        if (tid == 0) { s_ntouched = 0; s_nmerges = 0; s_nevents = m.E; s_stop = 0; }
        __syncthreads();
        for (uint32_t epoch = 1;; ++epoch) {
            int best = -1;
            for (uint32_t e = tid; e < m.E; e += MG_THREADS)
                if (m.ealive[e] && (best < 0 || edge_before(m, e, (uint32_t)best))) best = (int)e;
    #pragma unroll
            for (int d = 32; d >= 1; d >>= 1) {
                const int ob = __shfl_xor(best, d, 64);
                if (ob >= 0 && (best < 0 || edge_before(m, (uint32_t)ob, (uint32_t)best))) best = ob;
            }
            if (lane == 0) s_wbest[wave] = best;
            __syncthreads();
            if (tid == 0) {
                int b = -1;
                for (int w = 0; w < MG_THREADS / 64; ++w) { const int ob = s_wbest[w]; if (ob >= 0 && (b < 0 || edge_before(m, (uint32_t)ob, (uint32_t)b))) b = ob; }
                if (b < 0 || !(m.ew[b] < m.threshold)) s_stop = 1;
                else {
                    s_a = m.ea[b]; s_b = m.eb[b];
                    const uint32_t k = s_nmerges++;
                    m.merges[k * 3] = s_a; m.merges[k * 3 + 1] = s_b; m.merges[k * 3 + 2] = __float_as_uint(m.ew[b]);
                    m.ealive[b] = 0;
                }
            }
            __syncthreads();
            if (s_stop) break;
            const uint32_t a = s_a, b = s_b;
            if (wave == 0) {
                float acc = lane < 12 ? m.racc[(size_t)a * 12 + lane] : 0.0f;
                uint32_t cnt = m.rcnt[a];
                for (uint32_t leaf = m.rhead[b]; leaf; leaf = m.lnext[leaf]) {
                    const uint32_t off = m.loff[leaf], len = m.llen[leaf];
                    for (uint32_t j0 = 0; j0 < len; j0 += 16u) {
                        float val[16];
    #pragma unroll
                        for (int t = 0; t < 16; ++t) val[t] = (lane < 12 && j0 + t < len) ? m.rows[(size_t)(off + j0 + t) * 12 + lane] : 0.0f;
    #pragma unroll
                        for (int t = 0; t < 16; ++t)
                            if (j0 + t < len) {
                                cnt++;
                                if (lane < 9) acc += val[t];
                                else { const float count = (float)cnt; const float inv = 1 / count; acc = acc + inv * (val[t] - acc); }
                            }
                    }
                }
                if (lane < 12) m.racc[(size_t)a * 12 + lane] = acc;
                float all[12];
    #pragma unroll
                for (int k = 0; k < 12; ++k) all[k] = __shfl(acc, k, 64);
                float rec[16];
                a_region_from_acc(all, cnt, rec);
                if (lane == 0) {
                    for (int k = 0; k < 16; ++k) m.rrec[(size_t)a * 16 + k] = rec[k];
                    m.rcnt[a] = cnt;
                    m.lnext[m.rtail[a]] = m.rhead[b]; m.rtail[a] = m.rtail[b];
                    m.ralive[b] = 0; m.parent[b] = a;
                }
            } else {
                for (uint32_t e = tid - 64; e < m.E; e += MG_THREADS - 64) {
                    if (!m.ealive[e]) continue;
                    const uint32_t p = m.ea[e], q = m.eb[e];
                    const bool on_a = p == a || q == a, on_b = p == b || q == b;
                    if (!on_a && !on_b) continue;
                    const uint32_t x = (p == a || p == b) ? q : p;
                    m.tl[atomicAdd(&s_ntouched, 1u)] = e;
                    if (on_a) m.markA[x] = e + 1u; else m.markB[x] = e + 1u;
                }
            }
            __syncthreads();
            const uint32_t nt = s_ntouched;
            for (uint32_t i = tid; i < nt; i += MG_THREADS) {
                const uint32_t e = m.tl[i];
                const uint32_t p = m.ea[e], q = m.eb[e];
                const bool on_a = p == a || q == a;
                const uint32_t x = (p == a || p == b) ? q : p;
                const uint32_t partner = on_a ? m.markB[x] : m.markA[x];
                if (partner && edge_before(m, partner - 1u, e)) m.ealive[e] = 0;
            }
            __syncthreads();
            for (uint32_t i = tid; i < nt; i += MG_THREADS) {
                const uint32_t e = m.tl[i];
                const uint32_t p = m.ea[e], q = m.eb[e];
                const uint32_t x = (p == a || p == b) ? q : p;
                m.markA[x] = 0u; m.markB[x] = 0u;
                if (!m.ealive[e]) continue;
                const uint32_t lo = a < x ? a : x, hi = a < x ? x : a;
                int err = 0;
                const float w = a_edge_weight(mp, m.rrec + (size_t)lo * 16, m.rrec + (size_t)hi * 16, &err);
                if (err) m.dc->error = err;
                const uint32_t ev = atomicAdd(&s_nevents, 1u);
                if (ev >= m.ev_cap) { m.dc->error = F3DS_ERR_UNSUPPORTED; m.dc->ev_overflow = 1; continue; }
                const uint32_t ku = n_weight_key(w);
                m.ev_epoch[ev] = epoch; m.ev_key[ev] = ku; m.ev_prev[ev] = m.ehist[e];
                m.ea[e] = lo; m.eb[e] = hi; m.ew[e] = w; m.eku[e] = ku; m.ehist[e] = (int)ev;
            }
            if (tid == 0) s_ntouched = 0;
            __syncthreads();
            if (m.dc->error) break;
        }
        __syncthreads();
        if (tid == 0) { m.dc->n_merges = s_nmerges; m.dc->n_events = s_nevents; }
    }
};


constexpr uint32_t KEY_DEAD = 0xFFFFFFFFu;
constexpr uint32_t MC_TL_CAP = 1024;
constexpr uint32_t MC_LDS_LIMIT = 160u * 1024u - 2560u;
constexpr uint32_t MC_SP_TL = 256;
#ifndef F3DS_SP_REST_DIV
#define F3DS_SP_REST_DIV 4u
#endif
#ifndef F3DS_SP_ROWS8
#define F3DS_SP_ROWS8 1024u
#endif
#ifndef F3DS_SP_LEAVES
#define F3DS_SP_LEAVES 8
#endif
constexpr uint32_t MC_SP_LEAVES = F3DS_SP_LEAVES;
constexpr uint32_t MC_GROUP = 16;
struct MergeLds {
    uint2* pool; uint32_t pool_cap; uint32_t* rstart; uint32_t* rnleaf; uint32_t* rcap;
    uint32_t* ilist; uint32_t ilist_cap; uint32_t* istart; uint32_t* ilen; uint32_t* icap;
    uint32_t Ecap, NGcap, lds_bytes, stop_key;
    int keys_in_lds;
    int spec;
};
struct MergeIlLayout {
    uint32_t Ecap, NGcap, CH, sp_rows;
    uint32_t off_eab, off_akey, off_g1, off_dlist, off_dmask, off_tl, off_tx, off_hsh, off_lstart, off_lsrc, off_stage, off_stage2, total;
};
__host__ __device__ inline MergeIlLayout merge_il_offsets(uint32_t E, int nw, int res) {
    MergeIlLayout L;
    const uint32_t T = (uint32_t)nw * 64u;
    L.CH = nw == 4 ? 128u : 256u;
    L.Ecap = (E + 63u) & ~63u; if (!L.Ecap) L.Ecap = 64u;
    const uint32_t NG = L.Ecap / MC_GROUP;
    L.NGcap = (NG + T - 1u) / T * T;
    uint32_t o = 0u;
    L.off_eab = o; if (res == 2) o += L.Ecap * 4u;
    L.off_akey = o; if (res == 2) o += L.Ecap * 4u;
    L.off_g1 = o; o += L.NGcap * 4u;
    L.off_dlist = o; o += L.NGcap * 4u;
    L.off_dmask = o; o += ((L.NGcap + 31u) / 32u) * 4u;
    L.off_tl = o; o += MC_TL_CAP * 4u;
    L.off_tx = o; o += MC_TL_CAP * 4u;
    L.off_hsh = o; o += 2u * MC_TL_CAP * 4u;
    L.off_lstart = o; o += (T + 1u) * 4u;
    L.off_lsrc = o; o += T * 4u;
    o = (o + 15u) & ~15u;
    L.off_stage = o; o += 2u * L.CH * 52u + 64u;
    L.sp_rows = 128u;
    if (nw == 8) for (uint32_t r = F3DS_SP_ROWS8; r > 128u; r >>= 1) if (o + r * 52u + MC_SP_TL * 8u + 64u <= MC_LDS_LIMIT) { L.sp_rows = r; break; }
    L.off_stage2 = o; o += L.sp_rows * 52u + MC_SP_TL * 8u + 64u;
    L.total = o;
    return L;
}
struct d_inc_build {
    static constexpr bool LATENCY_KERNEL = true;
    static constexpr int BLOCK = 256;
    __device__ void operator()(uint32_t E, uint32_t S0, const uint32_t* ea, const uint32_t* eb, uint32_t* istart, uint32_t* ilen, uint32_t* icap, uint32_t* ilist) const {
        if (BIX) return;
        const uint32_t tid = threadIdx.x;
        for (uint32_t r = tid; r <= S0; r += BLOCK) icap[r] = 0u;
        __syncthreads();
        for (uint32_t e = tid; e < E; e += BLOCK) { atomicAdd(&icap[ea[e]], 1u); atomicAdd(&icap[eb[e]], 1u); }
        __syncthreads();
        uint32_t carry = 0u;
        for (uint32_t r0 = 0; r0 <= S0; r0 += BLOCK) {
            const uint32_t r = r0 + tid;
            const uint32_t d = r <= S0 ? __hip_atomic_load(&icap[r], __ATOMIC_RELAXED, __HIP_MEMORY_SCOPE_AGENT) : 0u;
            uint32_t tot;
            const uint32_t inc = block_incl_scan<BLOCK>(d, &tot);
            if (r <= S0) { istart[r] = carry + inc - d; ilen[r] = d; }
            carry += tot;
            __syncthreads();
        }
        for (uint32_t r = tid; r <= S0; r += BLOCK) icap[r] = 0u;
        __syncthreads();
        for (uint32_t e = tid; e < E; e += BLOCK) {
            const uint32_t a = ea[e], b = eb[e];
            ilist[istart[a] + atomicAdd(&icap[a], 1u)] = e;
            ilist[istart[b] + atomicAdd(&icap[b], 1u)] = e;
        }
        __syncthreads();
        for (uint32_t r = tid; r <= S0; r += BLOCK) icap[r] = ilen[r];
    }
};
__device__ inline uint32_t wave_min_u32(uint32_t v) {
#define F3DS_DPP_MIN(ctrl, rmask)                                                                          \
    { const uint32_t t_ = (uint32_t)__builtin_amdgcn_update_dpp((int)v, (int)v, ctrl, rmask, 0xF, false); v = t_ < v ? t_ : v; }
    F3DS_DPP_MIN(0xB1, 0xF)
    F3DS_DPP_MIN(0x4E, 0xF)
    F3DS_DPP_MIN(0x141, 0xF)
    F3DS_DPP_MIN(0x140, 0xF)
    F3DS_DPP_MIN(0x142, 0xA)
    F3DS_DPP_MIN(0x143, 0xC)
#undef F3DS_DPP_MIN
    return (uint32_t)__builtin_amdgcn_readlane((int)v, 63);
}
__device__ inline bool edge_before_k(const MergeDev& m, uint32_t e, uint32_t ke, uint32_t f, uint32_t kf) {
    EdgeHist H{m.ev_epoch, m.ev_key, m.ev_prev};
    return a_edge_before(H, e, ke, m.ehist[e], f, kf, m.ehist[f]);
}

__device__ inline bool edge_before_fast(const MergeDev& m, uint32_t e, uint32_t ke, uint32_t f, uint32_t kf) {
    if (ke != kf) return ke < kf;
    EdgeHist H{m.ev_epoch, m.ev_key, m.ev_prev};
    return a_edge_before(H, e, ke, m.ehist[e], f, kf, m.ehist[f]);
}
__device__ inline uint32_t row_min_u32(uint32_t v) {
#define F3DS_DPP_MIN(ctrl)                                                                          \
    { const uint32_t t_ = (uint32_t)__builtin_amdgcn_update_dpp((int)v, (int)v, ctrl, 0xF, 0xF, false); v = t_ < v ? t_ : v; }
    F3DS_DPP_MIN(0xB1) F3DS_DPP_MIN(0x4E) F3DS_DPP_MIN(0x141) F3DS_DPP_MIN(0x140)
#undef F3DS_DPP_MIN
    return v;
}
__device__ inline uint32_t wave_incl_scan_dpp(uint32_t v) {
#define F3DS_DPP_SHR_ADD(n) v += (uint32_t)__builtin_amdgcn_update_dpp(0, (int)v, 0x110 + (n), 0xF, 0xF, true);
    F3DS_DPP_SHR_ADD(1) F3DS_DPP_SHR_ADD(2) F3DS_DPP_SHR_ADD(4) F3DS_DPP_SHR_ADD(8)
#undef F3DS_DPP_SHR_ADD
    const uint32_t t0 = (uint32_t)__builtin_amdgcn_readlane((int)v, 15), t1 = (uint32_t)__builtin_amdgcn_readlane((int)v, 31), t2 = (uint32_t)__builtin_amdgcn_readlane((int)v, 47);
    const int row = lane_id() >> 4;
    return v + (row >= 1 ? t0 : 0u) + (row >= 2 ? t1 : 0u) + (row >= 3 ? t2 : 0u);
}
typedef float f2v __attribute__((ext_vector_type(2)));
typedef float f4v __attribute__((ext_vector_type(4)));
__device__ __forceinline__ uint32_t lds_addr(const float* p) { return (uint32_t)(uintptr_t)(__attribute__((address_space(3))) const float*)p; }
#define FOLD_ISSUE_SUM(S, arow) asm volatile("ds_read2_b32 %0, %4 offset1:12\n\tds_read2_b32 %1, %4 offset0:24 offset1:36\n\tds_read2_b32 %2, %4 offset0:48 offset1:60\n\tds_read2_b32 %3, %4 offset0:72 offset1:84" \
    : "=&v"(S##_0), "=&v"(S##_1), "=&v"(S##_2), "=&v"(S##_3) : "v"(arow))
#define FOLD_WAIT_SUM(S, n) asm volatile("s_waitcnt lgkmcnt(" #n ")" : "+v"(S##_0), "+v"(S##_1), "+v"(S##_2), "+v"(S##_3))
#define FOLD_ISSUE_COL(S, arow, ainv) asm volatile("ds_read2_b32 %0, %6 offset1:12\n\tds_read2_b32 %1, %6 offset0:24 offset1:36\n\tds_read2_b32 %2, %6 offset0:48 offset1:60\n\tds_read2_b32 %3, %6 offset0:72 offset1:84\n\tds_read_b128 %4, %7\n\tds_read_b128 %5, %7 offset:16" \
    : "=&v"(S##_0), "=&v"(S##_1), "=&v"(S##_2), "=&v"(S##_3), "=&v"(S##i0), "=&v"(S##i1) : "v"(arow), "v"(ainv))
#define FOLD_WAIT_COL(S, n) asm volatile("s_waitcnt lgkmcnt(" #n ")" : "+v"(S##_0), "+v"(S##_1), "+v"(S##_2), "+v"(S##_3), "+v"(S##i0), "+v"(S##i1))
#ifndef F3DS_MERGE_WPS4
#define F3DS_MERGE_WPS4 2
#endif
template <int NW, int RES>
struct d_merge_il_t {
    static constexpr bool IN_LDS = RES == 2;
    static constexpr int BLOCK = NW * 64;
#ifdef F3DS_MERGE_WPS
    static constexpr int WAVES_PER_SIMD = NW == 8 ? F3DS_MERGE_WPS : 2;
#else
    static constexpr int WAVES_PER_SIMD = NW == 4 ? F3DS_MERGE_WPS4 : 1;
#endif
    __device__ void operator()(MergeDev m, MergeLds x) const {
        static_assert(NW == 4 || NW == 8, "four or eight waves");
        constexpr uint32_t T = (uint32_t)BLOCK;
        constexpr uint32_t CH = NW == 4 ? 128u : 256u;
        extern __shared__ __attribute__((aligned(16))) unsigned char smem[];
        const MergeIlLayout L = merge_il_offsets(m.E, NW, RES);
        uint32_t* eab = IN_LDS ? reinterpret_cast<uint32_t*>(smem + L.off_eab) : reinterpret_cast<uint32_t*>(m.ew);
        uint32_t* akey = IN_LDS ? reinterpret_cast<uint32_t*>(smem + L.off_akey) : m.eku;
        uint32_t* G1 = reinterpret_cast<uint32_t*>(smem + L.off_g1);
        uint32_t* dlist = reinterpret_cast<uint32_t*>(smem + L.off_dlist);
        uint32_t* dmask = reinterpret_cast<uint32_t*>(smem + L.off_dmask);
        uint32_t* tl = reinterpret_cast<uint32_t*>(smem + L.off_tl);
        uint32_t* tx = reinterpret_cast<uint32_t*>(smem + L.off_tx);
        uint32_t* hsh = reinterpret_cast<uint32_t*>(smem + L.off_hsh);
        uint32_t* lstart = reinterpret_cast<uint32_t*>(smem + L.off_lstart);
        uint32_t* lsrc = reinterpret_cast<uint32_t*>(smem + L.off_lsrc);
        float* stage = reinterpret_cast<float*>(smem + L.off_stage);
        float* sinv = stage + 2u * CH * 12u;
        const uint32_t SPR = L.sp_rows;
        float* stage2 = reinterpret_cast<float*>(smem + L.off_stage2);
        float* sinv2 = stage2 + SPR * 12u;
        uint32_t* tl2 = reinterpret_cast<uint32_t*>(sinv2 + SPR);
        uint32_t* tx2 = tl2 + MC_SP_TL;
        __shared__ __attribute__((aligned(16))) uint32_t s_arg[8];
        __shared__ uint32_t s_nt2, s_cross, s_min1;
        __shared__ float s_rec2[16];
        __shared__ uint32_t s_nt, s_nevents, s_pool_end, s_ipool_end, s_best, s_ndirty;
        __shared__ int s_err;
        __shared__ float s_rec[16];
        __shared__ __attribute__((aligned(16))) double s_mtab[MC_COUNT];
        struct Cold { uint32_t* merges; unsigned char* ralive; uint32_t* parent; uint32_t* ev_epoch; uint32_t* ev_key; int* ev_prev; int* ehist; DevCounters* dc; };
        __shared__ Cold s_cold;
        const int tid = threadIdx.x, lane = lane_id(), wave = tid >> 6;
        MergeParams mp = m.mp;
        if (mp.merging == 1) mp.lambda = m.dc->lambda;
        for (uint32_t e = tid; e < L.Ecap; e += T) {
            if (IN_LDS) akey[e] = e < m.E ? m.eku[e] : KEY_DEAD;
            else if (e >= m.E) akey[e] = KEY_DEAD;
            eab[e] = e < m.E ? ((m.ea[e] << 16) | m.eb[e]) : 0xFFFFFFFFu;
        }
        for (uint32_t i = tid; i < 2u * MC_TL_CAP; i += T) hsh[i] = 0u;
        for (uint32_t i = tid; i < L.NGcap; i += T) G1[i] = KEY_DEAD;
        for (uint32_t i = tid; i < (L.NGcap + 31u) / 32u; i += T) dmask[i] = 0u;
        m_table_fill(s_mtab, tid, (int)T);
        if (wave < 2) __builtin_amdgcn_s_setprio(3);
        if (tid == 0) { s_nt = 0; s_nevents = m.E; s_err = 0; s_pool_end = m.S0 + 1u; s_ipool_end = 2u * m.E; s_ndirty = 0u; s_nt2 = 0u; s_cross = 0u; s_min1 = KEY_DEAD; }
        if (tid == 0) { s_cold.merges = m.merges; s_cold.ralive = m.ralive; s_cold.parent = m.parent; s_cold.ev_epoch = m.ev_epoch; s_cold.ev_key = m.ev_key; s_cold.ev_prev = m.ev_prev; s_cold.ehist = m.ehist; s_cold.dc = m.dc; }
        const uint32_t ev_cap = m.ev_cap;
        uint32_t nmerges = 0;
        __syncthreads();
        auto rescan = [&](const uint32_t count, const bool from_list) {
            const uint32_t row = (uint32_t)lane >> 4, l16 = (uint32_t)lane & 15u;
            for (uint32_t base = (uint32_t)wave * 4u; base < count; base += (uint32_t)NW * 4u) {
                const uint32_t i = base + row;
                const bool valid = i < count;
                const uint32_t g = valid ? (from_list ? dlist[i] : i) : 0u;
                const uint32_t k = valid ? akey[g * MC_GROUP + l16] : KEY_DEAD;
                const uint32_t m1 = row_min_u32(k);
                if (valid && l16 == 0u) {
                    G1[g] = m1;
                    if (from_list) atomicAnd(&dmask[g >> 5], ~(1u << (g & 31u)));
                }
            }
        };
        auto mark_dirty = [&](const uint32_t e) {
            const uint32_t g = e / MC_GROUP, bit = 1u << (g & 31u);
            if (!(atomicOr(&dmask[g >> 5], bit) & bit)) dlist[atomicAdd(&s_ndirty, 1u)] = g;
        };
        auto key_changed = [&](const uint32_t e, const uint32_t kold, const uint32_t knew) {
            uint32_t* gp = &G1[e / MC_GROUP];
            const uint32_t g1 = *gp;
            if (knew < g1) atomicMin(gp, knew);
            else if (kold == g1) mark_dirty(e);
        };
        rescan(L.Ecap / MC_GROUP, false);
        __syncthreads();
    #ifdef F3DS_MERGE_PROF
        unsigned long long tph[16] = {0, 0, 0, 0, 0, 0, 0, 0, 0, 0, 0, 0, 0, 0, 0, 0}, tlast = __builtin_amdgcn_s_memtime(), tph_nt = 0, tph_rows = 0, tph_slow = 0, tph_geo = 0, tph_lab = 0, tph_nd = 0;
        unsigned long long sp_cand = 0, sp_disjoint = 0, sp_small = 0, sp_scan = 0, sp_ok = 0, sp_epochs = 0;
        unsigned long long cls_n[4] = {0, 0, 0, 0}, cls_rows[4] = {0, 0, 0, 0}, cls_fold[4] = {0, 0, 0, 0}, cls_all[4] = {0, 0, 0, 0}, cls_prev_rows = 0, cls_prev_fold = 0, cls_prev_all = 0, cls_prev_w = 0, cls_prev_scan = 0;
        unsigned long long cle_n[4] = {0, 0, 0, 0}, cle_nt[4] = {0, 0, 0, 0}, cle_w[4] = {0, 0, 0, 0}, cle_scan[4] = {0, 0, 0, 0}, cle_all[4] = {0, 0, 0, 0};
        const unsigned long long loop_u0 = __builtin_amdgcn_s_memtime(), loop_w0 = __builtin_amdgcn_s_memrealtime();
    #define TPH(i) do { if (tid == 0) { const unsigned long long now_ = __builtin_amdgcn_s_memtime(); tph[i] += now_ - tlast; tlast = now_; } } while (0)
    #else
    #define TPH(i) do { } while (0)
    #endif
        constexpr bool SPEC = true;
        const bool spec_on = SPEC && x.spec != 0;
        uint32_t sp_try = 0u, sp_hit = 0u, sp_rest = 0u;
        for (uint32_t epoch = 1;; ++epoch) {
#ifdef F3DS_EXP_DUP_A
            for (int dup_ = 0; dup_ < 2; ++dup_) {
#endif
            {
                const uint32_t nd = s_ndirty;
    #ifdef F3DS_MERGE_PROF
                if (tid == 0) { tph_nd += nd; TPH(15); }
    #endif
                rescan(nd, true);
            }
            TPH(11);
            __syncthreads();
            TPH(12);
#ifndef F3DS_EXP_DUP_A
            if (tid == 0) s_ndirty = 0u;
#endif
            if constexpr (SPEC) { if (sp_rest) sp_rest--; }
            if (wave == 0) {
                uint32_t kloc = KEY_DEAD, gloc = 0u, tieloc = 0u;
                uint32_t k2loc = KEY_DEAD, g2loc = 0u, k3loc = KEY_DEAD;
                for (uint32_t g0 = (uint32_t)lane; g0 < L.NGcap; g0 += 256u) {
                    uint32_t mm[4];
            #pragma unroll
                    for (int u = 0; u < 4; ++u) { const uint32_t g = g0 + 64u * (uint32_t)u; mm[u] = G1[g < L.NGcap ? g : g0]; }
            #pragma unroll
                    for (int u = 0; u < 4; ++u) {
                        const uint32_t g = g0 + 64u * (uint32_t)u;
                        if (g >= L.NGcap) break;
                        const uint32_t m4 = mm[u];
                        if constexpr (SPEC) {
                            const bool lt1 = m4 < kloc, lt2 = m4 < k2loc, lt3 = m4 < k3loc;
                            k3loc = lt2 ? k2loc : (lt3 ? m4 : k3loc);
                            g2loc = lt1 ? gloc : (lt2 ? g : g2loc); k2loc = lt1 ? kloc : (lt2 ? m4 : k2loc);
                        }
                        if (m4 == kloc) tieloc = 1u;
                        if (m4 < kloc) { kloc = m4; gloc = g; tieloc = 0u; }
                    }
                }
                const uint32_t kmin_ = wave_min_u32(kloc);
                const uint64_t hit = __ballot(kloc == kmin_);
                const int src = __builtin_ctzll(hit);
                const uint32_t gbest = (uint32_t)__builtin_amdgcn_readlane((int)gloc, src);
                uint32_t tie_ = ((hit & (hit - 1ull)) != 0ull || (__ballot(tieloc != 0u) & hit) != 0ull) ? 1u : 0u;
                const bool want2 = SPEC && spec_on && !tie_ && sp_rest == 0u && kmin_ < x.stop_key;
                uint32_t q2 = KEY_DEAD, g2 = 0u, q3 = KEY_DEAD;
                if (want2) {
                    const uint32_t o2 = lane == src ? k2loc : kloc, og2 = lane == src ? g2loc : gloc;
                    q2 = wave_min_u32(o2);
                    const int src2 = __builtin_ctzll(__ballot(o2 == q2));
                    g2 = (uint32_t)__builtin_amdgcn_readlane((int)og2, src2);
                    const uint32_t o3 = lane == src ? (lane == src2 ? k3loc : k2loc) : (lane == src2 ? k2loc : kloc);
                    q3 = wave_min_u32(o3);
                }
                const uint32_t row = (uint32_t)lane >> 4, l16 = (uint32_t)lane & 15u;
                const bool rowon = row == 0u || (row == 1u && want2);
                const uint32_t slot0 = (row == 0u ? gbest : g2) * MC_GROUP + l16;
                const uint32_t kk0 = rowon ? akey[slot0] : KEY_DEAD;
                const uint32_t abrow = rowon ? eab[slot0] : 0u;
                const uint32_t m1 = row_min_u32(kk0);
                const uint32_t bits1 = (uint32_t)(__ballot(kk0 == m1) >> (row * 16u)) & 0xFFFFu;
                const uint32_t pos1 = (uint32_t)__builtin_ctz(bits1 | 0x10000u);
                const uint32_t kk1 = l16 == pos1 ? KEY_DEAD : kk0;
                const uint32_t m2 = row_min_u32(kk1);
                const uint32_t bits2 = (uint32_t)(__ballot(kk1 == m2) >> (row * 16u)) & 0xFFFFu;
                const uint32_t pos2 = (uint32_t)__builtin_ctz(bits2 | 0x10000u) & 15u;
                const uint32_t dup2 = (m2 != KEY_DEAD && __popc(bits2) >= 2) ? 1u : 0u;
                const uint32_t c2 = (uint32_t)__builtin_amdgcn_readlane((int)m2, 0), p1 = (uint32_t)__builtin_amdgcn_readlane((int)pos1, 0), p2 = (uint32_t)__builtin_amdgcn_readlane((int)pos2, 0);
                const uint32_t d2 = (uint32_t)__builtin_amdgcn_readlane((int)dup2, 0);
                if (c2 == kmin_) tie_ = 1u;
                const uint32_t best_ = gbest * MC_GROUP + p1;
                uint32_t best2_ = 0u, kmin2_ = KEY_DEAD, spec_ = 0u, lane2_ = 0u;
                if (want2 && !tie_) {
                    const uint32_t r_c2 = (uint32_t)__builtin_amdgcn_readlane((int)m2, 16), r_p1 = (uint32_t)__builtin_amdgcn_readlane((int)pos1, 16);
                    bool unique = false;
                    if (c2 < q2) { kmin2_ = c2; best2_ = gbest * MC_GROUP + p2; lane2_ = p2; unique = d2 == 0u; }
                    else if (q2 < c2) { kmin2_ = q2; best2_ = g2 * MC_GROUP + r_p1; lane2_ = 16u + r_p1; unique = r_c2 != q2 && q3 != q2; }
                    spec_ = (unique && kmin2_ > kmin_ && kmin2_ < x.stop_key) ? 1u : 0u;
                }
                const uint32_t ab_ = (uint32_t)__builtin_amdgcn_readlane((int)abrow, (int)p1), ab2_ = spec_ ? (uint32_t)__builtin_amdgcn_readlane((int)abrow, (int)lane2_) : 0u;
                if (lane == 0) { s_arg[0] = kmin_; s_arg[1] = best_; s_arg[2] = tie_; s_arg[3] = spec_; s_arg[4] = best2_; s_arg[5] = kmin2_; s_arg[6] = ab_; s_arg[7] = ab2_; }
            }
            TPH(13);
            __syncthreads();
            TPH(14);
#ifdef F3DS_EXP_DUP_A
            }
            if (tid == 0) s_ndirty = 0u;
#endif
            const uint4 arg0 = *reinterpret_cast<const uint4*>(&s_arg[0]), arg1 = *reinterpret_cast<const uint4*>(&s_arg[4]);
            const uint32_t kmin = (uint32_t)__builtin_amdgcn_readfirstlane((int)arg0.x);
            if (!(kmin < x.stop_key)) break;
            uint32_t best = (uint32_t)__builtin_amdgcn_readfirstlane((int)arg0.y);
            const uint32_t tie = (uint32_t)__builtin_amdgcn_readfirstlane((int)arg0.z);
            bool spec = __builtin_amdgcn_readfirstlane((int)arg0.w) != 0;
            const uint32_t best2 = (uint32_t)__builtin_amdgcn_readfirstlane((int)arg1.x), kmin2 = (uint32_t)__builtin_amdgcn_readfirstlane((int)arg1.y);
    #ifdef F3DS_MERGE_PROF
            if (spec) sp_cand++;
    #endif
            if (tie) {
                for (uint32_t e = tid; e < L.Ecap; e += T)
                    if (akey[e] == kmin) { const uint32_t i = atomicAdd(&s_nt, 1u); if (i < MC_TL_CAP) tl[i] = e; }
                __syncthreads();
                const uint32_t nc = s_nt;
                if (nc > MC_TL_CAP) { if (tid == 0) s_cold.dc->error = F3DS_ERR_UNSUPPORTED; break; }
                if (tid == 0) {
                    uint32_t bb = tl[0];
                    for (uint32_t i = 1; i < nc; ++i) { const uint32_t f = tl[i]; if (a_edge_before(EdgeHist{s_cold.ev_epoch, s_cold.ev_key, s_cold.ev_prev}, f, kmin, s_cold.ehist[f], bb, kmin, s_cold.ehist[bb])) bb = f; }
                    s_best = bb; s_nt = 0u;
                }
                __syncthreads();
                best = s_best;
    #ifdef F3DS_MERGE_PROF
                tph_slow++;
    #endif
            }
            TPH(0);
            const uint32_t ab_best = tie ? eab[best] : (uint32_t)__builtin_amdgcn_readfirstlane((int)arg1.z);
            const uint32_t a = ab_best >> 16, b = ab_best & 0xFFFFu;
            uint32_t a2 = 0u, b2 = 0u;
            if constexpr (SPEC) {
                if (spec) {
                    const uint32_t ab2 = (uint32_t)__builtin_amdgcn_readfirstlane((int)arg1.w);
                    a2 = ab2 >> 16; b2 = ab2 & 0xFFFFu;
                    if (a2 == a || a2 == b || b2 == a || b2 == b) spec = false;
                    if (spec) sp_try++;
    #ifdef F3DS_MERGE_PROF
                    if (spec) sp_disjoint++;
    #endif
                }
            }
            if (tid == 0) {
                const uint32_t wb = (kmin & 0x80000000u) ? (kmin & 0x7fffffffu) : ~kmin;
                uint32_t* mg = s_cold.merges; mg[nmerges * 3u] = a; mg[nmerges * 3u + 1u] = b; mg[nmerges * 3u + 2u] = wb;
            }
            nmerges++;
            const uint32_t a_start = x.rstart[a], na = x.rnleaf[a], cap_a = x.rcap[a], b_start = x.rstart[b], nb = x.rnleaf[b];
            const uint32_t cnt_a = m.rcnt[a];
            const uint32_t il_a = x.istart[a], il_na = x.ilen[a], il_ca = x.icap[a], il_b = x.istart[b], il_nb = x.ilen[b];
            const uint32_t b_off0 = m.loff[b], b_len0 = m.llen[b];
            uint32_t v_a2s = 0u, v_na2 = 0u, v_cnt2 = 0u, v_cap2 = 0u, v_nb2 = 0u, v_b2s = 0u, v_rows2 = 0u;
            uint32_t v_il_a2 = 0u, v_il_na2 = 0u, v_il_ca2 = 0u, v_il_b2 = 0u, v_il_nb2 = 0u;
            uint2 v_leaf2 = make_uint2(0u, 0u);
            if constexpr (SPEC) {
                if (spec) {
                    uint32_t vz;
                    asm volatile("v_mov_b32 %0, 0" : "=v"(vz));
                    v_a2s = x.rstart[a2 + vz]; v_na2 = x.rnleaf[a2 + vz]; v_cnt2 = m.rcnt[a2 + vz]; v_cap2 = x.rcap[a2 + vz]; v_nb2 = x.rnleaf[b2 + vz];
                    v_leaf2 = make_uint2(m.loff[b2 + vz], m.llen[b2 + vz]);
                    v_b2s = x.rstart[b2 + vz]; v_rows2 = m.rcnt[b2 + vz];
                    v_il_a2 = x.istart[a2 + vz]; v_il_na2 = x.ilen[a2 + vz]; v_il_ca2 = x.icap[a2 + vz]; v_il_b2 = x.istart[b2 + vz]; v_il_nb2 = x.ilen[b2 + vz];
                }
            }
            float acc = 0.0f;
            if (wave == 0 && lane < 9) acc = m.racc[(size_t)a * 12 + lane];
            if (wave == 1 && lane < 3) acc = m.racc[(size_t)a * 12 + 9 + lane];
            if constexpr (SPEC) {
                if (spec && wave == 2 && lane < 9) acc = m.racc[(size_t)a2 * 12 + lane];
                if (spec && wave == 3 && lane < 3) acc = m.racc[(size_t)a2 * 12 + 9 + lane];
            }
            const uint2 leaf0 = (uint32_t)tid < nb ? x.pool[b_start + tid] : make_uint2(0u, 0u);
            TPH(5);
            auto walk = [&](const uint32_t i0, const uint32_t stride, const uint32_t sA, const uint32_t lA, const uint32_t sB, const uint32_t lB, const uint32_t pa, const uint32_t pb,
                            const uint32_t skip, const uint32_t second, const uint32_t oa, const uint32_t ob) {
                const uint32_t n = lA + lB;
                for (uint32_t base = 0; base < n; base += stride) {
                    const uint32_t i = base + i0;
                    uint32_t e = 0u, ab = 0xFFFFFFFFu;
                    if (i < n) { e = x.ilist[i < lA ? sA + i : sB + (i - lA)]; ab = eab[e]; }
                    const bool hit = ab != 0xFFFFFFFFu && e != skip;
                    const uint32_t p = ab >> 16, q = ab & 0xFFFFu;
                    const bool on_a = p == pa || q == pa;
                    const uint32_t xx = (p == pa || p == pb) ? q : p;
                    if (hit && (xx == oa || xx == ob)) s_cross = 1u;
                    const uint64_t hm = __ballot(hit);
                    if (hm == 0ull) continue;
                    uint32_t wbase = 0u;
                    if (lane == 0) wbase = atomicAdd(second ? &s_nt2 : &s_nt, (uint32_t)__popcll(hm));
                    wbase = (uint32_t)__builtin_amdgcn_readfirstlane((int)wbase);
                    const uint32_t idx = wbase + (uint32_t)__popcll(hm & lanemask_lt());
                    if (hit && idx < (second ? MC_SP_TL : MC_TL_CAP)) {
                        (second ? tl2 : tl)[idx] = e; (second ? tx2 : tx)[idx] = xx | (on_a ? 0u : 0x80000000u);
                        const uint32_t hk = ((xx << 2) | (second << 1) | (on_a ? 0u : 1u)) + 1u;
                        for (uint32_t sl = (hk * 2654435761u) >> 21;; sl = (sl + 1u) & (2u * MC_TL_CAP - 1u))
                            if (atomicCAS(&hsh[sl], 0u, (hk << 10) | idx) == 0u) break;
                    }
                }
            };
            if (SPEC && spec) {
                if ((uint32_t)tid < T / 2u) walk((uint32_t)tid, T / 2u, il_a, il_na, il_b, il_nb, a, b, best, 0u, a2, b2);
                else walk((uint32_t)tid - T / 2u, T / 2u, v_il_a2, v_il_na2, v_il_b2, v_il_nb2, a2, b2, best2, 1u, 0xFFFFFFFFu, 0xFFFFFFFFu);
            } else walk((uint32_t)tid, T, il_a, il_na, il_b, il_nb, a, b, best, 0u, 0xFFFFFFFFu, 0xFFFFFFFFu);
            TPH(6);
            const bool in_place = na + nb <= cap_a;
            const uint32_t new_start = in_place ? a_start : s_pool_end;
            const uint32_t new_cap = in_place ? cap_a : 2u * (na + nb);
            if (!in_place && new_start + new_cap > x.pool_cap) { if (tid == 0) { DevCounters* dcp = s_cold.dc; dcp->error = F3DS_ERR_UNSUPPORTED; dcp->ev_overflow = 2; } break; }
            if (in_place) { for (uint32_t i = tid; i < nb; i += T) x.pool[a_start + na + i] = i < T ? leaf0 : x.pool[b_start + i]; }
            else { for (uint32_t i = tid; i < na + nb; i += T) x.pool[new_start + i] = i < na ? x.pool[a_start + i] : x.pool[b_start + (i - na)]; }
            TPH(7);
            __syncthreads();
            TPH(1);
            const uint32_t nt = (uint32_t)__builtin_amdgcn_readfirstlane((int)s_nt);
            uint32_t nt2 = 0u;
            uint32_t a2_start = 0u, na2 = 0u, cnt_a2 = 0u, cap_a2 = 0u, nb2 = 0u, il_a2 = 0u, il_ca2 = 0u, b2_start = 0u, rows2 = 0u;
            uint2 leaf2 = make_uint2(0u, 0u);
            if constexpr (SPEC) {
                if (spec) {
                    nt2 = (uint32_t)__builtin_amdgcn_readfirstlane((int)s_nt2);
                    if (s_cross != 0u || nt2 > MC_SP_TL || nt + nt2 > T) spec = false;
    #ifdef F3DS_MERGE_PROF
                    if (spec) sp_scan++;
    #endif
                }
                if (spec) {
                    a2_start = (uint32_t)__builtin_amdgcn_readfirstlane((int)v_a2s); na2 = (uint32_t)__builtin_amdgcn_readfirstlane((int)v_na2); cnt_a2 = (uint32_t)__builtin_amdgcn_readfirstlane((int)v_cnt2);
                    cap_a2 = (uint32_t)__builtin_amdgcn_readfirstlane((int)v_cap2); nb2 = (uint32_t)__builtin_amdgcn_readfirstlane((int)v_nb2);
                    leaf2.x = (uint32_t)__builtin_amdgcn_readfirstlane((int)v_leaf2.x); leaf2.y = (uint32_t)__builtin_amdgcn_readfirstlane((int)v_leaf2.y);
                    il_a2 = (uint32_t)__builtin_amdgcn_readfirstlane((int)v_il_a2); il_ca2 = (uint32_t)__builtin_amdgcn_readfirstlane((int)v_il_ca2);
                    b2_start = (uint32_t)__builtin_amdgcn_readfirstlane((int)v_b2s);
                    rows2 = nb2 == 1u ? leaf2.y : (uint32_t)__builtin_amdgcn_readfirstlane((int)v_rows2);
                    if (nb2 == 0u || nb2 > MC_SP_LEAVES || rows2 > SPR || rows2 == 0u) spec = false;
    #ifdef F3DS_MERGE_PROF
                    if (spec) sp_small++;
    #endif
                }
            }
            bool in_place2 = true; uint32_t new_start2 = 0u, new_cap2 = 0u;
            if constexpr (SPEC) {
                if (spec) {
                    in_place2 = na2 + nb2 <= cap_a2;
                    new_start2 = in_place2 ? a2_start : s_pool_end + (in_place ? 0u : new_cap);
                    new_cap2 = in_place2 ? cap_a2 : 2u * (na2 + nb2);
                    if (!in_place2 && new_start2 + new_cap2 > x.pool_cap) spec = false;
// ... 159 lines not shown
                            FOLD_WAIT_SUM(B, 0);
                            FOLD_TAIL_SUM(B, left - la);
    #undef FOLD_TAIL_SUM
                        }
                    };
                    auto fold_colour = [&](const float* buf, const float* bi, const uint32_t nr) {
                        if (lane < 3) {
                            uint32_t arow = lds_addr(buf + 9 + lane), ainv = lds_addr(bi);
                            f2v A_0, A_1, A_2, A_3, B_0, B_1, B_2, B_3;
                            f4v Ai0, Ai1, Bi0, Bi1;
    #define FOLD_STEP(c, i) acc = acc + (i) * ((c) - acc)
    #define FOLD_EIGHT(S) do { FOLD_STEP(S##_0.x, S##i0.x); FOLD_STEP(S##_0.y, S##i0.y); FOLD_STEP(S##_1.x, S##i0.z); FOLD_STEP(S##_1.y, S##i0.w); \
                               FOLD_STEP(S##_2.x, S##i1.x); FOLD_STEP(S##_2.y, S##i1.y); FOLD_STEP(S##_3.x, S##i1.z); FOLD_STEP(S##_3.y, S##i1.w); } while (0)
                            FOLD_ISSUE_COL(A, arow, ainv); arow += 8u * 48u; ainv += 32u;
                            uint32_t j = 0;
                            for (; j + 16u <= nr; j += 16u) {
                                FOLD_ISSUE_COL(B, arow, ainv); arow += 8u * 48u; ainv += 32u;
                                FOLD_WAIT_COL(A, 6);
                                FOLD_EIGHT(A);
                                FOLD_ISSUE_COL(A, arow, ainv); arow += 8u * 48u; ainv += 32u;
                                FOLD_WAIT_COL(B, 6);
                                FOLD_EIGHT(B);
                            }
    #define FOLD_TAIL_COL(S, r) do { if ((r) > 0u) FOLD_STEP(S##_0.x, S##i0.x); if ((r) > 1u) FOLD_STEP(S##_0.y, S##i0.y); if ((r) > 2u) FOLD_STEP(S##_1.x, S##i0.z); if ((r) > 3u) FOLD_STEP(S##_1.y, S##i0.w); \
                                     if ((r) > 4u) FOLD_STEP(S##_2.x, S##i1.x); if ((r) > 5u) FOLD_STEP(S##_2.y, S##i1.y); if ((r) > 6u) FOLD_STEP(S##_3.x, S##i1.z); if ((r) > 7u) FOLD_STEP(S##_3.y, S##i1.w); } while (0)
                            const uint32_t left = nr - j, la = left < 8u ? left : 8u;
                            FOLD_ISSUE_COL(B, arow, ainv);
                            FOLD_WAIT_COL(A, 6);
                            FOLD_TAIL_COL(A, la);
                            FOLD_WAIT_COL(B, 0);
                            FOLD_TAIL_COL(B, left - la);
    #undef FOLD_TAIL_COL
    #undef FOLD_EIGHT
    #undef FOLD_STEP
                        }
                    };
#ifdef F3DS_EXP_DUP_F
                    { const float acc0 = acc;
                      if (wave == 0) fold_sums(buf, nr); else if (wave == 1) fold_colour(buf, bi, nr);
                      float t_ = acc; asm volatile("" : "+v"(t_)); acc = acc0 + (t_ - t_); }
#endif
                    if (wave == 0) fold_sums(buf, nr);
                    else if (wave == 1) fold_colour(buf, bi, nr);
                    else if (fold2_here) {
                        const uint32_t nr2 = (uint32_t)__builtin_amdgcn_readfirstlane((int)rows2);
                        if (wave == 2) fold_sums(stage2, nr2); else fold_colour(stage2, sinv2, nr2);
                        if (more && load_later && rn < Tl) load_row(rn);
                    }
                    rows_done += nr;
                    if (more && loader && rn < Tl) store_row((c + 1u) & 1u, ld, cnt_a + rows_done + ld + 1u);
                    __syncthreads();
                }
    #ifdef F3DS_MERGE_PROF
                if (tid == 0) tph_rows += Tl;
    #endif
            }
            TPH(2);
            if (wave == 0 && lane < 9) m.racc[(size_t)a * 12 + lane] = acc;
            if (wave == 1 && lane < 3) m.racc[(size_t)a * 12 + 9 + lane] = acc;
            const uint32_t npre = (NW > 2 && !(SPEC && spec && T <= 256u)) ? (nt < 2u * CH ? nt : 2u * CH) : 0u;
            auto record_geometry = [&](const uint32_t cnt, float* srec, const bool commit) {
    #ifdef F3DS_MERGE_PROF
                const unsigned long long tg0 = __builtin_amdgcn_s_memtime();
    #endif
                float cen[3], n4[4];
                const m_lds mc = m_lds_here(s_mtab);
                if (cnt >= 3u) plane_normal_wave(acc, cnt, lane, cen, n4, mc);
                else {
                    float all[9];
    #pragma unroll
                    for (int k = 0; k < 9; ++k) all[k] = wave_pick(acc, k);
                    const float c = (float)cnt;
                    cen[0] = all[6] / c; cen[1] = all[7] / c; cen[2] = all[8] / c;
                    n_plane_normal(all, cnt, cen, n4);
                }
    #ifdef F3DS_MERGE_PROF
                if (tid == 0) tph_geo += __builtin_amdgcn_s_memtime() - tg0;
    #endif
                if (lane == 0) {
                    for (int k = 0; k < 3; ++k) { srec[k] = cen[k]; srec[3 + k] = n4[k]; }
                    if (commit) {
                        for (int k = 0; k < 3; ++k) { m.rrec[(size_t)a * 16 + k] = cen[k]; m.rrec[(size_t)a * 16 + 3 + k] = n4[k]; }
                        m.rcnt[a] = cnt;
                        x.rstart[a] = new_start; x.rnleaf[a] = na + nb; x.rcap[a] = new_cap; if (!in_place) s_pool_end = new_start + new_cap;
                        x.istart[a] = il_new; x.ilen[a] = nt; x.icap[a] = il_newcap; if (!il_in_place) s_ipool_end = il_new + il_newcap;
                        s_cold.ralive[b] = 0; s_cold.parent[b] = a;
                    }
                }
            };
            auto record_colour = [&](float* srec, const bool commit) {
    #ifdef F3DS_MERGE_PROF
                const unsigned long long tc0 = __builtin_amdgcn_s_memtime();
    #endif
                const float mr = __int_as_float(__builtin_amdgcn_readlane(__float_as_int(acc), 0)), mg = __int_as_float(__builtin_amdgcn_readlane(__float_as_int(acc), 1)),
                            mb = __int_as_float(__builtin_amdgcn_readlane(__float_as_int(acc), 2));
                float lab[3];
                const m_lds mc = m_lds_here(s_mtab);
                lab_three_lanes(lane == 0 ? mr : (lane == 1 ? mg : mb), lane, lab, mc);
                if (lane == 0) {
                    const float rec[6] = {mr, mg, mb, lab[0], lab[1], lab[2]};
                    for (int k = 0; k < 6; ++k) { srec[6 + k] = rec[k]; if (commit) m.rrec[(size_t)a * 16 + 6 + k] = rec[k]; }
    #ifdef F3DS_MERGE_PROF
                    if (commit) s_rec[12] = (float)(__builtin_amdgcn_s_memtime() - tc0);
    #endif
                }
            };
            auto prefetch_far_ends = [&](uint32_t first, uint32_t step) {
                for (uint32_t i = first; i < npre; i += step) {
                    if (tx[i] & 0x40000000u) continue;
                    const float4* gx = reinterpret_cast<const float4*>(m.rrec + (size_t)(tx[i] & 0xFFFFu) * 16);
                    const float4 x0 = gx[0], x1 = gx[1], x2 = gx[2];
                    float4* dst = reinterpret_cast<float4*>(stage + (size_t)i * 12);
                    dst[0] = x0; dst[1] = x1; dst[2] = x2;
                }
            };
            auto publish_edge = [&](uint32_t e, uint32_t lo, uint32_t hi, int hprev, uint32_t ku, uint32_t ep, uint32_t kold) {
                const uint32_t ev = atomicAdd(&s_nevents, 1u);
                if (ev >= ev_cap) { DevCounters* dcp = s_cold.dc; dcp->error = F3DS_ERR_UNSUPPORTED; dcp->ev_overflow = 1; s_err = 1; return; }
                s_cold.ev_epoch[ev] = ep; s_cold.ev_key[ev] = ku; s_cold.ev_prev[ev] = hprev;
                s_cold.ehist[e] = (int)ev;
                akey[e] = ku; eab[e] = (lo << 16) | hi;
                key_changed(e, kold, ku);
            };
            if (!(SPEC && spec)) rows2 = 0u;
#ifdef F3DS_EXP_DUP_R
            if (wave == 0) record_geometry(cnt_a + rows_done, s_rec, true);
            else if (wave == 1) record_colour(s_rec, true);
#endif
            if (wave == 0) record_geometry(cnt_a + rows_done, s_rec, true);
            else if (wave == 1) record_colour(s_rec, true);
            else if (SPEC && spec && wave == 2) record_geometry(cnt_a2 + rows2, s_rec2, false);
            else if (SPEC && spec && wave == 3) record_colour(s_rec2, false);
            else if constexpr (NW > 2) {
                if (SPEC && spec) { if (T > 256u && wave >= 4) prefetch_far_ends((uint32_t)tid - 256u, T - 256u); }
                else prefetch_far_ends((uint32_t)tid - 128u, T - 128u);
            }
            __syncthreads();
            TPH(3);
    #ifdef F3DS_MERGE_PROF
            if (tid == 0) tph_lab += (unsigned long long)s_rec[12];
    #endif
            const uint32_t ntw = nt + (SPEC && spec ? nt2 : 0u);
            const bool quad = NW > 2 && mp.color_metric == 0 && ntw * 4u <= (T < 256u ? T : 256u);
            const int qsh = quad ? 2 : 0;
            bool valid2 = false;
            if (SPEC && spec) {
                const uint32_t i = (uint32_t)tid >> qsh;
                const bool mine = i < ntw, second = mine && i >= nt;
                const bool lead = !quad || (lane & 3) == 0;
                uint32_t e = 0u, txi = 0x40000000u, ku = KEY_DEAD, lo = 0u, hi = 0u, kold = KEY_DEAD; int hprev = 0, err = 0;
                if (mine) {
                    const uint32_t j = second ? i - nt : i;
                    e = second ? tl2[j] : tl[j]; txi = second ? tx2[j] : tx[j];
                    kold = akey[e];
                }
                if (mine && !(txi & 0x40000000u)) {
                    const uint32_t xx = txi & 0xFFFFu, ra = second ? a2 : a;
                    lo = ra < xx ? ra : xx; hi = ra < xx ? xx : ra;
                    float r1[12], r2[12];
                    hprev = s_cold.ehist[e];
                    {
                        const float4* gx = (!second && i < npre) ? reinterpret_cast<const float4*>(stage + (size_t)i * 12) : reinterpret_cast<const float4*>(m.rrec + (size_t)xx * 16);
                        const float4 x0 = gx[0], x1 = gx[1], x2 = gx[2];
                        const float rx[12] = {x0.x, x0.y, x0.z, x0.w, x1.x, x1.y, x1.z, x1.w, x2.x, x2.y, x2.z, x2.w};
                        const bool a_first = ra < xx;
                        const float* sr = second ? s_rec2 : s_rec;
    #pragma unroll
                        for (int k = 0; k < 12; ++k) { const float rr = sr[k]; r1[k] = a_first ? rr : rx[k]; r2[k] = a_first ? rx[k] : rr; }
                    }
                    const m_lds mc = m_lds_here(s_mtab);
#ifdef F3DS_EXP_DUP_W
                    { const float w0 = quad ? edge_weight_quad(mp, r1, r2, lane & 3, &err, mc) : a_edge_weight(mp, r1, r2, &err, mc); r1[9] += (w0 - w0); }
#endif
                    const float w = quad ? edge_weight_quad(mp, r1, r2, lane & 3, &err, mc) : a_edge_weight(mp, r1, r2, &err, mc);
                    ku = n_weight_key(w);
                    if (lead && !second) atomicMin(&s_min1, ku);
                }
                __syncthreads();
                valid2 = s_min1 > kmin2;
                if (mine && lead && (!second || valid2)) {
                    if (txi & 0x40000000u) { akey[e] = KEY_DEAD; eab[e] = 0xFFFFFFFFu; key_changed(e, kold, KEY_DEAD); }
                    else {
                        if (err) { s_cold.dc->error = err; s_err = 1; }
                        publish_edge(e, lo, hi, hprev, ku, second ? epoch + 1u : epoch, kold);
                    }
                }
            } else {
                for (uint32_t i = (uint32_t)tid >> qsh; i < nt; i += T >> qsh) {
                    const uint32_t e = tl[i], txi = tx[i];
                    const uint32_t xx = txi & 0xFFFFu;
                    const uint32_t kold = akey[e];
                    const bool lead = !quad || (lane & 3) == 0;
                    if (txi & 0x40000000u) { if (lead) { akey[e] = KEY_DEAD; eab[e] = 0xFFFFFFFFu; key_changed(e, kold, KEY_DEAD); } continue; }
                    const uint32_t lo = a < xx ? a : xx, hi = a < xx ? xx : a;
                    float r1[12], r2[12];
                    const int hprev = s_cold.ehist[e];
                    {
                        const float4* gx = i < npre ? reinterpret_cast<const float4*>(stage + (size_t)i * 12) : reinterpret_cast<const float4*>(m.rrec + (size_t)xx * 16);
                        const float4 x0 = gx[0], x1 = gx[1], x2 = gx[2];
                        const float rx[12] = {x0.x, x0.y, x0.z, x0.w, x1.x, x1.y, x1.z, x1.w, x2.x, x2.y, x2.z, x2.w};
                        const bool a_first = a < xx;
    #pragma unroll
                        for (int k = 0; k < 12; ++k) { const float ra = s_rec[k]; r1[k] = a_first ? ra : rx[k]; r2[k] = a_first ? rx[k] : ra; }
                    }
                    int err = 0;
                    const m_lds mc = m_lds_here(s_mtab);
#ifdef F3DS_EXP_DUP_W
                    { const float w0 = quad ? edge_weight_quad(mp, r1, r2, lane & 3, &err, mc) : a_edge_weight(mp, r1, r2, &err, mc); r1[9] += (w0 - w0); }
#endif
                    const float w = quad ? edge_weight_quad(mp, r1, r2, lane & 3, &err, mc) : a_edge_weight(mp, r1, r2, &err, mc);
                    if (lead) {
                        if (err) { s_cold.dc->error = err; s_err = 1; }
                        publish_edge(e, lo, hi, hprev, n_weight_key(w), epoch, kold);
                    }
                }
            }
            if (tid == 0) { s_nt = 0; akey[best] = KEY_DEAD; eab[best] = 0xFFFFFFFFu; mark_dirty(best); }
            if constexpr (SPEC) {
                if (spec) {
                    if (valid2) {
                        if (wave == 2 && lane < 9) m.racc[(size_t)a2 * 12 + lane] = acc;
                        if (wave == 3 && lane < 3) m.racc[(size_t)a2 * 12 + 9 + lane] = acc;
                        if (tid == 128) {
                            for (int k = 0; k < 12; ++k) m.rrec[(size_t)a2 * 16 + k] = s_rec2[k];
                            m.rcnt[a2] = cnt_a2 + rows2;
                            x.rstart[a2] = new_start2; x.rnleaf[a2] = na2 + nb2; x.rcap[a2] = new_cap2; if (!in_place2) s_pool_end = new_start2 + new_cap2;
                            s_cold.ralive[b2] = 0; s_cold.parent[b2] = a2;
                            const uint32_t wb2 = (kmin2 & 0x80000000u) ? (kmin2 & 0x7fffffffu) : ~kmin2;
                            uint32_t* mg = s_cold.merges; mg[nmerges * 3u] = a2; mg[nmerges * 3u + 1u] = b2; mg[nmerges * 3u + 2u] = wb2;
                            akey[best2] = KEY_DEAD; eab[best2] = 0xFFFFFFFFu; mark_dirty(best2);
                            x.istart[a2] = il_new2; x.ilen[a2] = nt2; x.icap[a2] = il_newcap2; if (!il_in_place2) s_ipool_end = il_new2 + il_newcap2;
                        }
                        for (uint32_t i = tid; i < nt2; i += T) x.ilist[il_new2 + i] = tl2[i];
                        nmerges++; epoch++; sp_hit++;
    #ifdef F3DS_MERGE_PROF
                        sp_ok++;
    #endif
                    }
                    if (tid == 0) { s_nt2 = 0u; s_cross = 0u; s_min1 = KEY_DEAD; }
                } else if (tid == 0 && (s_nt2 | s_cross)) { s_nt2 = 0u; s_cross = 0u; }
            }
            if (SPEC && sp_try >= 64u) { if (sp_hit * F3DS_SP_REST_DIV < sp_try) sp_rest = 256u; sp_try = 0u; sp_hit = 0u; }
            for (uint32_t i = tid; i < 2u * MC_TL_CAP; i += T) hsh[i] = 0u;
            __syncthreads();
            TPH(4);
    #ifdef F3DS_MERGE_PROF
            sp_epochs++;
            if (tid == 0) {
                unsigned long long all_ = 0; for (int k = 0; k < 16; ++k) all_ += tph[k];
                const uint32_t rc = tph_rows - cls_prev_rows < 32 ? 0 : (tph_rows - cls_prev_rows < 256 ? 1 : (tph_rows - cls_prev_rows < 1024 ? 2 : 3));
                const uint32_t ec = nt <= 16 ? 0 : (nt <= 64 ? 1 : (nt <= 256 ? 2 : 3));
                cls_n[rc] += 1; cls_rows[rc] += tph_rows - cls_prev_rows; cls_fold[rc] += (tph[2] + tph[10] + tph[9] + tph[8]) - cls_prev_fold; cls_all[rc] += all_ - cls_prev_all;
                cle_n[ec] += 1; cle_nt[ec] += nt; cle_w[ec] += tph[4] - cls_prev_w; cle_scan[ec] += (tph[6] + tph[0]) - cls_prev_scan; cle_all[ec] += all_ - cls_prev_all;
                cls_prev_rows = tph_rows; cls_prev_fold = tph[2] + tph[10] + tph[9] + tph[8]; cls_prev_all = all_; cls_prev_w = tph[4]; cls_prev_scan = tph[6] + tph[0];
                tlast = __builtin_amdgcn_s_memtime();
            }
    #endif
            if (s_err) break;
        }
        __syncthreads();
        if (tid == 0) { DevCounters* dcp = s_cold.dc; dcp->n_merges = nmerges; dcp->n_events = s_nevents; }
    #ifdef F3DS_MERGE_PROF
        if (tid == 0 && f3ds_frame() == 0) {
            const double nm = nmerges ? (double)nmerges : 1.0;
            { const unsigned long long loop_u1 = __builtin_amdgcn_s_memtime(), loop_w1 = __builtin_amdgcn_s_memrealtime();
              printf("  whole loop: %.0f shader clocks, %.1f per tick of the 100 MHz clock (%.2f ms)\n", (double)(loop_u1 - loop_u0), (double)(loop_u1 - loop_u0) / (double)(loop_w1 - loop_w0), (double)(loop_w1 - loop_w0) * 1e-5); }
            printf("d_merge_il<%d,%d> cycles/merge: argmin (dirty groups + group minima) %.0f [log+meta %.0f list walk %.0f pool %.0f barrier %.0f] [leaves %.0f load+dedupe+store %.0f barrier %.0f fold %.0f] record %.0f weights %.0f  (merges %u, touched/merge %.1f, rows/merge %.1f, tie slow paths %llu)\n",
                   NW, RES, (double)(tph[0] + tph[11] + tph[12] + tph[13] + tph[14] + tph[15]) / nm, (double)tph[5] / nm, (double)tph[6] / nm, (double)tph[7] / nm, (double)tph[1] / nm, (double)tph[8] / nm, (double)tph[9] / nm, (double)tph[10] / nm, (double)tph[2] / nm, (double)tph[3] / nm, (double)tph[4] / nm, nmerges, (double)tph_nt / nm, (double)tph_rows / nm, tph_slow);
            printf("  argmin phase: epoch head %.0f, dirty-group rescan %.0f (%.1f groups per epoch), barrier %.0f, wave 0: group-minima argmin + runner-up %.0f, barrier %.0f, rest %.0f\n", (double)tph[15] / nm, (double)tph[11] / nm, (double)tph_nd / (double)sp_epochs, (double)tph[12] / nm, (double)tph[13] / nm, (double)tph[14] / nm, (double)tph[0] / nm);
            printf("  record: wave 0 (centroid, normal) %.0f cycles/merge, wave 1 (Lab) %.0f\n", (double)tph_geo / nm, (double)tph_lab / nm);
            printf("  speculation: %llu epochs for %u merges; runner-up unique and below the threshold %llu, regions disjoint %llu, second merge small enough %llu, no joining edge %llu, committed %llu\n", sp_epochs, nmerges, sp_cand, sp_disjoint, sp_small, sp_scan, sp_ok);
            for (int k = 0; k < 4; ++k) printf("  rows class %d (<32, <256, <1024, more): %llu merges, %llu rows, leaves+load+fold %.0f cycles/merge = %.1f per row, whole merge %.0f\n", k, cls_n[k], cls_rows[k], cls_n[k] ? (double)cls_fold[k] / cls_n[k] : 0.0, cls_rows[k] ? (double)cls_fold[k] / cls_rows[k] : 0.0, cls_n[k] ? (double)cls_all[k] / cls_n[k] : 0.0);
            for (int k = 0; k < 4; ++k) printf("  touched class %d (<=16, <=64, <=256, more): %llu merges, %llu edges, weights %.0f cycles/merge = %.1f per edge, argmin+scan %.0f, whole merge %.0f\n", k, cle_n[k], cle_nt[k], cle_n[k] ? (double)cle_w[k] / cle_n[k] : 0.0, cle_nt[k] ? (double)cle_w[k] / cle_nt[k] : 0.0, cle_n[k] ? (double)cle_scan[k] / cle_n[k] : 0.0, cle_n[k] ? (double)cle_all[k] / cle_n[k] : 0.0);
        }
    #endif
    #undef TPH
    }
};

#ifdef F3DS_WHATIF
struct d_fake_merge {
    static constexpr int BLOCK = 512;
    __device__ void operator()(MergeDev m, uint32_t us, uint32_t waves) const {
        extern __shared__ uint32_t fm_lds[];
        if (threadIdx.x == 0) { fm_lds[0] = 0u; m.dc->n_merges = 0u; m.dc->n_events = 0u; }
        if ((threadIdx.x >> 6) < waves) {
            const unsigned long long t0 = __builtin_amdgcn_s_memrealtime();
            while (__builtin_amdgcn_s_memrealtime() - t0 < (unsigned long long)us * 100ull) __builtin_amdgcn_s_sleep(64);
        }
        __syncthreads();
    }
};
#endif

__device__ inline void relabel_tables(uint32_t S0, const uint32_t* parent, const unsigned char* ralive, uint32_t* rank, bool writer,
                                      uint32_t* root_out, uint32_t* incl_out, DevCounters* dc) {
    __shared__ uint32_t rl_wtot[4];
    const uint32_t lane = (uint32_t)lane_id(), w = threadIdx.x >> 6;
    uint32_t carry = 0;
    for (uint32_t base = 0; base <= S0; base += 256u) {
        const uint32_t h = base + threadIdx.x;
        const bool alive = h > 0u && h <= S0 && ralive[h] != 0;
        const uint64_t mask = __ballot(alive);
        const uint32_t within = __builtin_amdgcn_mbcnt_hi((uint32_t)(mask >> 32), __builtin_amdgcn_mbcnt_lo((uint32_t)mask, 0u));
        if (lane == 0u) rl_wtot[w] = (uint32_t)__popcll(mask);
        __syncthreads();
        uint32_t before = 0, total = 0;
#pragma unroll
        for (uint32_t k = 0; k < 4u; ++k) { const uint32_t t = rl_wtot[k]; total += t; if (k < w) before += t; }
        const uint32_t incl = carry + before + within + (alive ? 1u : 0u);
        if (h <= S0) {
            rank[h] = alive ? incl - 1u : F3DS_NO_LABEL;
            if (writer) incl_out[h] = incl;
        }
        carry += total;
        __syncthreads();
    }
    if (writer && threadIdx.x == 0) dc->n_regions = carry;
    for (uint32_t h = threadIdx.x; h <= S0; h += 256u) {
        uint32_t r = h;
        while (parent[r] != r) r = parent[r];
        if (writer) root_out[h] = r;
        if (r != h) rank[h] = rank[r];
    }
    __syncthreads();
}
__device__ inline void relabel_points(uint32_t n, const int* pt_voxel, const uint32_t* owner, const uint32_t* rank, uint32_t* labels) {
    for (uint32_t i = BIX * blockDim.x + threadIdx.x; i < n; i += gridDim.x * blockDim.x) {
        const int v = pt_voxel[i];
        const uint32_t o = owner[v >= 0 ? v : 0];
        labels[i] = (v >= 0 && o) ? rank[o] : F3DS_NO_LABEL;
    }
}
constexpr uint32_t RL_LDS_CAP = 12288;
struct d_relabel {
    static constexpr int BLOCK = 256;
    __device__ void operator()(uint32_t n, const int* pt_voxel, const uint32_t* owner, uint32_t S0, const uint32_t* parent, const unsigned char* ralive,
                               uint32_t* root_out, uint32_t* incl_out, uint32_t* labels, DevCounters* dc) const {
        extern __shared__ uint32_t rl_rank[];
        if (BIX > 0 && BIX * blockDim.x >= n) return;
        relabel_tables(S0, parent, ralive, rl_rank, BIX == 0, root_out, incl_out, dc);
        relabel_points(n, pt_voxel, owner, rl_rank, labels);
    }
};
struct d_region_ids {
    static constexpr int BLOCK = 256;
    __device__ void operator()(uint32_t S0, const uint32_t* parent, const unsigned char* ralive, uint32_t* rank, uint32_t* root_out, uint32_t* incl_out, DevCounters* dc) const {
        if (BIX) return;
        relabel_tables(S0, parent, ralive, rank, true, root_out, incl_out, dc);
    }
};
struct d_point_labels {
    static constexpr int BLOCK = 256;
// ... 101 lines not shown
```

Measured before the change: 3716.

## Pack per-region merge bookkeeping into 32-byte records and adapt merge kind to occupancy

```diff
diff --git a/fast-3d-pointcloud-segmentation_amd/csrc/f3ds_algo.h b/fast-3d-pointcloud-segmentation_amd/csrc/f3ds_algo.h
--- a/fast-3d-pointcloud-segmentation_amd/csrc/f3ds_algo.h
+++ b/fast-3d-pointcloud-segmentation_amd/csrc/f3ds_algo.h
@@ -504,5 +504,30 @@
     }
 }
 
+struct RegionBook { uint32_t rstart, rnleaf, rcap, rcnt, istart, ilen, icap, spare; };
+constexpr uint32_t RB_WORDS = 8u;
+enum { RB_RSTART = 0, RB_RNLEAF = 1, RB_RCAP = 2, RB_RCNT = 3, RB_ISTART = 4, RB_ILEN = 5, RB_ICAP = 6, RB_SPARE = 7 };
+F3DS_HD void a_book_pack(const RegionBook& r, uint32_t w[8]) {
+    w[RB_RSTART] = r.rstart; w[RB_RNLEAF] = r.rnleaf; w[RB_RCAP] = r.rcap; w[RB_RCNT] = r.rcnt;
+    w[RB_ISTART] = r.istart; w[RB_ILEN] = r.ilen; w[RB_ICAP] = r.icap; w[RB_SPARE] = r.spare;
+}
+F3DS_HD RegionBook a_book_unpack(const uint32_t w[8]) {
+    RegionBook r;
+    r.rstart = w[RB_RSTART]; r.rnleaf = w[RB_RNLEAF]; r.rcap = w[RB_RCAP]; r.rcnt = w[RB_RCNT];
+    r.istart = w[RB_ISTART]; r.ilen = w[RB_ILEN]; r.icap = w[RB_ICAP]; r.spare = w[RB_SPARE];
+    return r;
+}
+
+F3DS_HD int a_merge_kind_for(uint32_t frames, int calls_on_device, int calls_before_merge, uint32_t merge_frames_in_flight, uint32_t compute_units, unsigned fits, int shared_res) {
+    bool shared = frames >= 16u && calls_on_device >= 2;
+    if (shared && calls_before_merge <= 0 && (uint64_t)frames + merge_frames_in_flight <= compute_units) shared = false;
+    const int wide = shared ? 2 : 0;
+    for (int res = shared ? (shared_res == 2 ? 2 : 0) : 2; res >= 0; res -= 2) {
+        const int k = wide + (res == 2 ? 0 : 1);
+        if (fits & (1u << k)) return 1 + k;
+    }
+    return 0;
+}
+
 }
 #endif
diff --git a/fast-3d-pointcloud-segmentation_amd/csrc/f3ds_hip.hip b/fast-3d-pointcloud-segmentation_amd/csrc/f3ds_hip.hip
--- a/fast-3d-pointcloud-segmentation_amd/csrc/f3ds_hip.hip
+++ b/fast-3d-pointcloud-segmentation_amd/csrc/f3ds_hip.hip
@@ -102,6 +102,7 @@
 };
 thread_local Switches g_sw;
 const int g_merge_shared_res = [] { const char* e = dev_getenv("F3DS_MERGE_SHARED_RES"); return e && atoi(e) == 2 ? 2 : 0; }();
+const bool g_merge_lone_tail = [] { const char* e = dev_getenv("F3DS_MERGE_LONE_TAIL"); return !(e && atoi(e) == 0); }();
 
 #define F3DS_SCRATCH(X) \
     X(P16, pts) X(P16, spts) X(uint64_t, keys0) X(uint64_t, keys1) X(uint32_t, vals0) X(uint32_t, vals1) X(uint32_t, flags) X(uint32_t, incl) X(uint32_t, tiles) X(uint32_t, hist) X(uint32_t, seg_start) X(int, pt_voxel) X(uint32_t, labels) \
@@ -114,7 +115,7 @@
      X(uint32_t, glut) X(uint32_t, truth_pts) X(uint32_t, tsum) X(uint32_t, tcol) X(uint32_t, tlab) X(uint32_t, ctab) X(uint32_t, csize) X(uint32_t, eroot) X(uint32_t, eincl) \
      X(uint32_t, hcnt) X(uint32_t, pslot) X(uint32_t, vlist) \
      X(uint32_t, u_src) X(uint32_t, u_voff) X(float, u_xyz) X(uint32_t, u_rgba) X(float, u_cent) X(float, u_nrm) \
-    X(float, deltas) X(uint64_t, skeys0) X(uint64_t, skeys1) X(uint32_t, svals0) X(uint32_t, svals1) X(uint32_t, cdf_hist) X(float, cdf) X(uint32_t, root) X(uint32_t, rincl) X(uint32_t, rrank) X(uint2, pool) X(uint32_t, rstart) X(uint32_t, rnleaf) X(uint32_t, rcap) X(uint32_t, tile_n1) X(uint32_t, tile_ord) X(uint32_t, tile_slots) X(uint32_t, ilist) X(uint32_t, istart) X(uint32_t, ilen) X(uint32_t, icap) \
+    X(float, deltas) X(uint64_t, skeys0) X(uint64_t, skeys1) X(uint32_t, svals0) X(uint32_t, svals1) X(uint32_t, cdf_hist) X(float, cdf) X(uint32_t, root) X(uint32_t, rincl) X(uint32_t, rrank) X(uint2, pool) X(uint32_t, rbook) X(uint32_t, tile_n1) X(uint32_t, tile_ord) X(uint32_t, tile_slots) X(uint32_t, ilist) \
      X(uint32_t, lv_into) X(uint32_t, lv_at) X(uint32_t, lv_pfx) X(float, lv_thr) X(uint32_t, lv_tab) X(uint32_t, lv_nreg) X(uint32_t, lv_out)
 template <class T> struct Scratch { T* p = nullptr; size_t cap = 0; int slot = -1; };
 #define F3DS_SCRATCH_SLOT(T, name) S_##name,
@@ -240,6 +241,26 @@
 thread_local int g_batch_frames = 1;
 std::atomic<int> g_batch_calls[16];
 struct BatchCallCount { int d; explicit BatchCallCount(int dev) : d(dev & 15) { g_batch_calls[d].fetch_add(1, std::memory_order_relaxed); } ~BatchCallCount() { g_batch_calls[d].fetch_sub(1, std::memory_order_relaxed); } };
+std::atomic<int> g_calls_before_merge[16];
+std::atomic<int> g_merge_frames_in_flight[16];
+struct BeforeMergeCount {
+    int d; bool held = true;
+    explicit BeforeMergeCount(int dev) : d(dev & 15) { g_calls_before_merge[d].fetch_add(1, std::memory_order_relaxed); }
+    void done() { if (held) { held = false; g_calls_before_merge[d].fetch_sub(1, std::memory_order_relaxed); } }
+    ~BeforeMergeCount() { done(); }
+};
+struct MergeFramesInFlight {
+    int d = 0, n = 0;
+    void raise(int dev, size_t frames) { drop(); d = dev & 15; n = (int)frames; g_merge_frames_in_flight[d].fetch_add(n, std::memory_order_relaxed); }
+    void drop() { if (n) { g_merge_frames_in_flight[d].fetch_sub(n, std::memory_order_relaxed); n = 0; } }
+    ~MergeFramesInFlight() { drop(); }
+};
+uint32_t compute_units_of(int device) {
+    static std::atomic<int> cu[16];
+    int v = cu[device & 15].load(std::memory_order_relaxed);
+    if (!v) { if (hipDeviceGetAttribute(&v, hipDeviceAttributeMultiprocessorCount, device) != hipSuccess || v < 1) { (void)hipGetLastError(); v = 1; } cu[device & 15].store(v, std::memory_order_relaxed); }
+    return (uint32_t)v;
+}
 size_t grid_cap_for_batch(int frames) {
     static const size_t target = dev_getenv("F3DS_GRID_TARGET") ? (size_t)atol(dev_getenv("F3DS_GRID_TARGET")) : 3072;
     if (!target) return 2048;
@@ -297,6 +318,7 @@
     std::vector<f3ds_ctx*> fr;
     hipStream_t st = nullptr;
     f3ds_ctx* owner = nullptr;
+    BeforeMergeCount* ahead = nullptr;
 };
 
 thread_local double g_t_wait = 0, g_t_launch = 0;
@@ -670,17 +692,20 @@
 inline int mk_waves(int kind) { return (kind - MK_IL) >= 2 ? 4 : 8; }
 inline int mk_res(int kind) { return (kind - MK_IL) % 2 ? 0 : 2; }
 int choose_merge_kind(const std::vector<f3ds_ctx*>& fr, bool force_global) {
-    if (force_global || g_sw.force_global_merge) return MK_GLOBAL;
-    const bool e_keys = g_sw.merge_keys >= 0;
-    const bool shared = fr.size() >= 16 && g_batch_calls[fr[0]->device & 15].load(std::memory_order_relaxed) >= 2;
-    const int nw = g_sw.merge_nw ? (g_sw.merge_nw == 8 ? 8 : 4) : (shared ? 4 : 8);
-    const int first = e_keys ? (g_sw.merge_keys == 2 ? 2 : 0) : (shared ? g_merge_shared_res : 2);
-    for (int res = first; res >= (e_keys ? first : 0); res -= 2) {
+    if (force_global || g_sw.force_global_merge || fr.empty()) return MK_GLOBAL;
+    auto nw_of = [](int kind) { return g_sw.merge_nw ? (g_sw.merge_nw == 8 ? 8 : 4) : mk_waves(kind); };
+    auto res_of = [](int kind) { return g_sw.merge_keys >= 0 ? (g_sw.merge_keys == 2 ? 2 : 0) : mk_res(kind); };
+    unsigned fits = 0u;
+    for (int k = 0; k < 4; ++k) {
         bool ok = true;
-        for (f3ds_ctx* c : fr) { MergeLds t; if (!merge_il_layout(c->E, c->S0, nw, res, &t)) { ok = false; break; } }
-        if (ok) return MK_IL + (nw == 8 ? 0 : 2) + (res == 2 ? 0 : 1);
-    }
-    return MK_GLOBAL;
+        for (f3ds_ctx* c : fr) { MergeLds t; if (!merge_il_layout(c->E, c->S0, nw_of(MK_IL + k), res_of(MK_IL + k), &t)) { ok = false; break; } }
+        if (ok) fits |= 1u << k;
+    }
+    const int d = fr[0]->device & 15;
+    const int kind = a_merge_kind_for((uint32_t)fr.size(), g_batch_calls[d].load(std::memory_order_relaxed), g_merge_lone_tail ? g_calls_before_merge[d].load(std::memory_order_relaxed) : 1,
+                                      (uint32_t)std::max(0, g_merge_frames_in_flight[d].load(std::memory_order_relaxed)), compute_units_of(fr[0]->device), fits, g_merge_shared_res);
+    if (kind == MK_GLOBAL) return MK_GLOBAL;
+    return MK_IL + (nw_of(kind) == 8 ? 0 : 2) + (res_of(kind) == 2 ? 0 : 1);
 }
 int seg_cluster_front(f3ds_ctx* c, const f3ds_params* prm, int kind) {
     const bool use_lds = kind != MK_GLOBAL;
@@ -713,19 +738,18 @@
     merge_il_layout(E, S0, use_lds ? mk_waves(kind) : 8, use_lds ? mk_res(kind) : 0, &xl);
     uint32_t logS = 1; while ((1u << logS) < S0 + 2u) ++logS;
     xl.pool_cap = (S0 + 1u) * (4u * logS + 8u) * c->pool_mult;
-    ENSURE(c->pool, xl.pool_cap, xl.pool); ENSURE(c->rstart, S0 + 1, xl.rstart); ENSURE(c->rnleaf, S0 + 1, xl.rnleaf);
-    ENSURE(c->rcap, S0 + 1, xl.rcap);
+    ENSURE(c->pool, xl.pool_cap, xl.pool); ENSURE(c->rbook, (size_t)(S0 + 1) * RB_WORDS, xl.book);
     if (use_lds) {
         const uint64_t bound = 2ull * E + (uint64_t)(S0 ? S0 - 1u : 0u) * (MC_TL_CAP + MC_TL_CAP / 2u + 4u) + 1024u;
         uint64_t cap = 2ull * E + (uint64_t)g_sw.ilist_slack * E * c->ilist_mult + (g_sw.ilist_slack < 32u ? 16u : 1024u);
         if (cap > bound) cap = bound;
         xl.ilist_cap = cap > 0x7fffffffull ? 0x7fffffffu : (uint32_t)cap;
-        ENSURE(c->ilist, xl.ilist_cap, xl.ilist); ENSURE(c->istart, S0 + 1, xl.istart); ENSURE(c->ilen, S0 + 1, xl.ilen); ENSURE(c->icap, S0 + 1, xl.icap);
-    }
-    if (use_lds) rec<d_inc_build>(c, 1u, 0u, E, S0, m.ea, m.eb, xl.istart, xl.ilen, xl.icap, xl.ilist);
+        ENSURE(c->ilist, xl.ilist_cap, xl.ilist);
+    }
+    if (use_lds) rec<d_inc_build>(c, 1u, 0u, E, S0, m.ea, m.eb, xl.book, xl.ilist);
     xl.stop_key = (prm->threshold != prm->threshold) ? 0u : n_weight_key(prm->threshold);
     c->merge_in_lds = use_lds; c->merge_kind = kind;
-    rec<d_region_reset>(c, grid_for(S0 + 1, 256), 0u, S0, c->hcount.p, m.rhead, m.rtail, m.lnext, m.parent, m.markA, m.markB, xl.pool, xl.rstart, xl.rnleaf, xl.rcap, c->loff.p);
+    rec<d_region_reset>(c, grid_for(S0 + 1, 256), 0u, S0, c->hcount.p, m.rhead, m.rtail, m.lnext, m.parent, m.markA, m.markB, xl.pool, xl.book, m.rcnt, c->loff.p);
     m.mp.color_metric = prm->color_metric; m.mp.geom_metric = prm->geom_metric; m.mp.merging = prm->merging; m.mp.lambda = lambda; m.mp.bins = bins;
     uint64_t *sk0 = nullptr, *sk1 = nullptr; uint32_t *sv0 = nullptr, *sv1 = nullptr;
     if (prm->merging == F3DS_ADAPTIVE_LAMBDA) {
@@ -836,12 +860,15 @@
 }
 
 int run_cluster(Batch& b, const f3ds_params* prm, uint32_t* const* labels_of, const std::vector<int>& index_of, int labels_on_device, bool force_global = false) {
+    if (b.ahead) b.ahead->done();
     const int kind = choose_merge_kind(b.fr, force_global);
+    MergeFramesInFlight in_flight;
     const bool all_lds = kind != MK_GLOBAL;
     int rc = for_frames(b, [&](f3ds_ctx* c) { return seg_cluster_front(c, prm, kind); });
     if (rc || (rc = flush(b))) return rc;
     stage_mark(b, 5);
     if ((rc = for_frames(b, seg_merge)) || (rc = flush(b))) return rc;
+    if (!b.fr.empty()) in_flight.raise(b.fr[0]->device, b.fr.size());
     stage_mark(b, 6);
     for (size_t i = 0; i < b.fr.size(); ++i) {
         uint32_t* out = labels_of ? labels_of[index_of[i]] : nullptr;
@@ -874,6 +901,7 @@
         }
         if (dl) HIPCHECK(hipEventRecord(b.owner->ev_copy[2], dl));
         if ((rc = flush_sync(b))) return rc;
+        in_flight.drop();
         if (dl) HIPCHECK(timed_sync(b.owner->ev_copy[2]));
     }
     {
@@ -991,8 +1019,9 @@
     g_sw.read();
     HIPCHECK(hipSetDevice(ctxs[0]->device));
     BatchCallCount in_flight(ctxs[0]->device);
+    BeforeMergeCount ahead(ctxs[0]->device);
     Batch b;
-    b.owner = ctxs[0]; b.st = ctxs[0]->stream;
+    b.owner = ctxs[0]; b.st = ctxs[0]->stream; b.ahead = &ahead;
     BatchStreamLease lease;
     if (nctx > 1 && ctxs[0]->stream == ctxs[0]->own_stream && !g_sw.no_stream_pool) { hipStream_t ps = lease.acquire(ctxs[0]->device); if (ps) b.st = ps; }
     g_grid_cap = grid_cap_for_batch(nctx); g_batch_frames = nctx;
@@ -1268,16 +1297,16 @@
 inline uint32_t label_out(const f3ds_ctx* c, uint32_t h) { return c->user_mode && h < c->user_label.size() ? c->user_label[h] : h; }
 int region_leaves(f3ds_ctx* c, std::vector<unsigned char>& ralive, std::vector<std::vector<uint2>>& leaves) {
     const uint32_t S0 = c->S0;
-    std::vector<uint32_t> rhead, lnext, loff, llen, rstart, rnleaf; std::vector<uint2> pool;
+    std::vector<uint32_t> rhead, lnext, loff, llen, book; std::vector<uint2> pool;
     int rc;
     if ((rc = fetch(c, c->ralive, S0 + 1, ralive)) || (rc = fetch(c, c->rhead, S0 + 1, rhead)) || (rc = fetch(c, c->lnext, S0 + 1, lnext)) ||
         (rc = fetch(c, c->loff, S0 + 2, loff)) || (rc = fetch(c, c->hcount, S0 + 1, llen)))
         return rc;
-    if (c->merge_in_lds && ((rc = fetch(c, c->pool, c->pool.cap / 8, pool)) || (rc = fetch(c, c->rstart, S0 + 1, rstart)) || (rc = fetch(c, c->rnleaf, S0 + 1, rnleaf)))) return rc;
+    if (c->merge_in_lds && ((rc = fetch(c, c->pool, c->pool.cap / 8, pool)) || (rc = fetch(c, c->rbook, (size_t)(S0 + 1) * RB_WORDS, book)))) return rc;
     leaves.assign(S0 + 1, {});
     for (uint32_t h = 1; h <= S0; ++h) {
         if (!ralive[h]) continue;
-        if (c->merge_in_lds) leaves[h].assign(pool.begin() + rstart[h], pool.begin() + rstart[h] + rnleaf[h]);
+        if (c->merge_in_lds) { const RegionBook r = a_book_unpack(&book[(size_t)h * RB_WORDS]); leaves[h].assign(pool.begin() + r.rstart, pool.begin() + r.rstart + r.rnleaf); }
         else for (uint32_t leaf = rhead[h]; leaf; leaf = lnext[leaf]) leaves[h].push_back(make_uint2(loff[leaf], llen[leaf]));
     }
     return F3DS_OK;
diff --git a/fast-3d-pointcloud-segmentation_amd/csrc/f3ds_kernels.inc b/fast-3d-pointcloud-segmentation_amd/csrc/f3ds_kernels.inc
--- a/fast-3d-pointcloud-segmentation_amd/csrc/f3ds_kernels.inc
+++ b/fast-3d-pointcloud-segmentation_amd/csrc/f3ds_kernels.inc
@@ -2811,12 +2811,13 @@
 struct d_region_reset {
     static constexpr int BLOCK = 256;
     __device__ void operator()(uint32_t S0, const uint32_t* hcount, uint32_t* rhead, uint32_t* rtail, uint32_t* lnext, uint32_t* parent,
-                                                     uint32_t* markA, uint32_t* markB, uint2* pool, uint32_t* rstart, uint32_t* rnleaf, uint32_t* rcap,
+                                                     uint32_t* markA, uint32_t* markB, uint2* pool, uint32_t* book, const uint32_t* rcnt,
                                                      const uint32_t* loff) const {
         for (uint32_t h = BIX * blockDim.x + threadIdx.x; h <= S0; h += gridDim.x * blockDim.x) {
             const bool alive = h > 0 && hcount[h] > 0;
             rhead[h] = alive ? h : 0u; rtail[h] = alive ? h : 0u; lnext[h] = 0u; parent[h] = h; markA[h] = 0u; markB[h] = 0u;
-            pool[h] = make_uint2(loff[h], hcount[h]); rstart[h] = h; rnleaf[h] = alive ? 1u : 0u; rcap[h] = 1u;
+            pool[h] = make_uint2(loff[h], hcount[h]);
+            *reinterpret_cast<uint4*>(book + (size_t)h * RB_WORDS) = make_uint4(h, alive ? 1u : 0u, 1u, rcnt[h]);
         }
     }
 };
@@ -2956,8 +2957,9 @@
 constexpr uint32_t MC_SP_LEAVES = F3DS_SP_LEAVES;
 constexpr uint32_t MC_GROUP = 16;
 struct MergeLds {
-    uint2* pool; uint32_t pool_cap; uint32_t* rstart; uint32_t* rnleaf; uint32_t* rcap;
-    uint32_t* ilist; uint32_t ilist_cap; uint32_t* istart; uint32_t* ilen; uint32_t* icap;
+    uint2* pool; uint32_t pool_cap;
+    uint32_t* book;
+    uint32_t* ilist; uint32_t ilist_cap;
     uint32_t Ecap, NGcap, lds_bytes, stop_key;
     int keys_in_lds;
     int spec;
@@ -2995,32 +2997,34 @@
 struct d_inc_build {
     static constexpr bool LATENCY_KERNEL = true;
     static constexpr int BLOCK = 256;
-    __device__ void operator()(uint32_t E, uint32_t S0, const uint32_t* ea, const uint32_t* eb, uint32_t* istart, uint32_t* ilen, uint32_t* icap, uint32_t* ilist) const {
+    __device__ void operator()(uint32_t E, uint32_t S0, const uint32_t* ea, const uint32_t* eb, uint32_t* book, uint32_t* ilist) const {
         if (BIX) return;
         const uint32_t tid = threadIdx.x;
-        for (uint32_t r = tid; r <= S0; r += BLOCK) icap[r] = 0u;
+        uint32_t *istart = book + RB_ISTART, *ilen = book + RB_ILEN, *icap = book + RB_ICAP;
+        constexpr uint32_t W = RB_WORDS;
+        for (uint32_t r = tid; r <= S0; r += BLOCK) icap[r * W] = 0u;
         __syncthreads();
-        for (uint32_t e = tid; e < E; e += BLOCK) { atomicAdd(&icap[ea[e]], 1u); atomicAdd(&icap[eb[e]], 1u); }
+        for (uint32_t e = tid; e < E; e += BLOCK) { atomicAdd(&icap[ea[e] * W], 1u); atomicAdd(&icap[eb[e] * W], 1u); }
         __syncthreads();
         uint32_t carry = 0u;
         for (uint32_t r0 = 0; r0 <= S0; r0 += BLOCK) {
             const uint32_t r = r0 + tid;
-            const uint32_t d = r <= S0 ? __hip_atomic_load(&icap[r], __ATOMIC_RELAXED, __HIP_MEMORY_SCOPE_AGENT) : 0u;
+            const uint32_t d = r <= S0 ? __hip_atomic_load(&icap[r * W], __ATOMIC_RELAXED, __HIP_MEMORY_SCOPE_AGENT) : 0u;
             uint32_t tot;
             const uint32_t inc = block_incl_scan<BLOCK>(d, &tot);
-            if (r <= S0) { istart[r] = carry + inc - d; ilen[r] = d; }
+            if (r <= S0) { istart[r * W] = carry + inc - d; ilen[r * W] = d; }
             carry += tot;
             __syncthreads();
         }
-        for (uint32_t r = tid; r <= S0; r += BLOCK) icap[r] = 0u;
+        for (uint32_t r = tid; r <= S0; r += BLOCK) icap[r * W] = 0u;
         __syncthreads();
         for (uint32_t e = tid; e < E; e += BLOCK) {
             const uint32_t a = ea[e], b = eb[e];
-            ilist[istart[a] + atomicAdd(&icap[a], 1u)] = e;
-            ilist[istart[b] + atomicAdd(&icap[b], 1u)] = e;
+            ilist[istart[a * W] + atomicAdd(&icap[a * W], 1u)] = e;
+            ilist[istart[b * W] + atomicAdd(&icap[b * W], 1u)] = e;
         }
         __syncthreads();
-        for (uint32_t r = tid; r <= S0; r += BLOCK) icap[r] = ilen[r];
+        for (uint32_t r = tid; r <= S0; r += BLOCK) { icap[r * W] = ilen[r * W]; book[r * W + RB_SPARE] = 0u; }
     }
 };
 __device__ inline uint32_t wave_min_u32(uint32_t v) {
@@ -3072,6 +3076,30 @@
 #ifndef F3DS_MERGE_WPS4
 #define F3DS_MERGE_WPS4 2
 #endif
+#ifndef F3DS_MERGE_OUTLINE_W
+#define F3DS_MERGE_OUTLINE_W 0
+#endif
+template <bool QUAD>
+__device__ __attribute__((noinline)) f2v merge_weight_outlined(MergeParams mp, f4v a0, f4v a1, f4v a2, f4v b0, f4v b1, f4v b2, int q, m_lds mc) {
+    const float r1[12] = {a0.x, a0.y, a0.z, a0.w, a1.x, a1.y, a1.z, a1.w, a2.x, a2.y, a2.z, a2.w};
+    const float r2[12] = {b0.x, b0.y, b0.z, b0.w, b1.x, b1.y, b1.z, b1.w, b2.x, b2.y, b2.z, b2.w};
+    int err = 0;
+    float w;
+    if constexpr (QUAD) w = edge_weight_quad(mp, r1, r2, q, &err, mc); else w = a_edge_weight(mp, r1, r2, &err, mc);
+    f2v o; o.x = w; o.y = __int_as_float(err);
+    return o;
+}
+__device__ __forceinline__ float merge_weight(const MergeParams& mp, const float* r1, const float* r2, bool quad, int q, int* err, m_lds mc) {
+#if F3DS_MERGE_OUTLINE_W
+    f4v a0 = {r1[0], r1[1], r1[2], r1[3]}, a1 = {r1[4], r1[5], r1[6], r1[7]}, a2 = {r1[8], r1[9], r1[10], r1[11]};
+    f4v b0 = {r2[0], r2[1], r2[2], r2[3]}, b1 = {r2[4], r2[5], r2[6], r2[7]}, b2 = {r2[8], r2[9], r2[10], r2[11]};
+    const f2v o = quad ? merge_weight_outlined<true>(mp, a0, a1, a2, b0, b1, b2, q, mc) : merge_weight_outlined<false>(mp, a0, a1, a2, b0, b1, b2, q, mc);
+    if (__float_as_int(o.y)) *err = __float_as_int(o.y);
+    return o.x;
+#else
+    return quad ? edge_weight_quad(mp, r1, r2, q, err, mc) : a_edge_weight(mp, r1, r2, err, mc);
+#endif
+}
 template <int NW, int RES>
 struct d_merge_il_t {
     static constexpr bool IN_LDS = RES == 2;
@@ -3158,7 +3186,7 @@
         rescan(L.Ecap / MC_GROUP, false);
         __syncthreads();
     #ifdef F3DS_MERGE_PROF
-        unsigned long long tph[16] = {0, 0, 0, 0, 0, 0, 0, 0, 0, 0, 0, 0, 0, 0, 0, 0}, tlast = __builtin_amdgcn_s_memtime(), tph_nt = 0, tph_rows = 0, tph_slow = 0, tph_geo = 0, tph_lab = 0, tph_nd = 0;
+        unsigned long long tph[16] = {0, 0, 0, 0, 0, 0, 0, 0, 0, 0, 0, 0, 0, 0, 0, 0}, tlast = __builtin_amdgcn_s_memtime(), tph_nt = 0, tph_rows = 0, tph_slow = 0, tph_geo = 0, tph_lab = 0, tph_nd = 0, tph_book = 0;
         unsigned long long sp_cand = 0, sp_disjoint = 0, sp_small = 0, sp_scan = 0, sp_ok = 0, sp_epochs = 0;
         unsigned long long cls_n[4] = {0, 0, 0, 0}, cls_rows[4] = {0, 0, 0, 0}, cls_fold[4] = {0, 0, 0, 0}, cls_all[4] = {0, 0, 0, 0}, cls_prev_rows = 0, cls_prev_fold = 0, cls_prev_all = 0, cls_prev_w = 0, cls_prev_scan = 0;
         unsigned long long cle_n[4] = {0, 0, 0, 0}, cle_nt[4] = {0, 0, 0, 0}, cle_w[4] = {0, 0, 0, 0}, cle_scan[4] = {0, 0, 0, 0}, cle_all[4] = {0, 0, 0, 0};
@@ -3306,9 +3334,12 @@
                 uint32_t* mg = s_cold.merges; mg[nmerges * 3u] = a; mg[nmerges * 3u + 1u] = b; mg[nmerges * 3u + 2u] = wb;
             }
             nmerges++;
-            const uint32_t a_start = x.rstart[a], na = x.rnleaf[a], cap_a = x.rcap[a], b_start = x.rstart[b], nb = x.rnleaf[b];
-            const uint32_t cnt_a = m.rcnt[a];
-            const uint32_t il_a = x.istart[a], il_na = x.ilen[a], il_ca = x.icap[a], il_b = x.istart[b], il_nb = x.ilen[b];
+            const uint4* bk_a = reinterpret_cast<const uint4*>(x.book + (size_t)a * RB_WORDS);
+            const uint4* bk_b = reinterpret_cast<const uint4*>(x.book + (size_t)b * RB_WORDS);
+            const uint4 ra0 = bk_a[0], ra1 = bk_a[1], rb0 = bk_b[0], rb1 = bk_b[1];
+            const uint32_t a_start = ra0.x, na = ra0.y, cap_a = ra0.z, b_start = rb0.x, nb = rb0.y;
+            const uint32_t cnt_a = ra0.w;
+            const uint32_t il_a = ra1.x, il_na = ra1.y, il_ca = ra1.z, il_b = rb1.x, il_nb = rb1.y;
             const uint32_t b_off0 = m.loff[b], b_len0 = m.llen[b];
             uint32_t v_a2s = 0u, v_na2 = 0u, v_cnt2 = 0u, v_cap2 = 0u, v_nb2 = 0u, v_b2s = 0u, v_rows2 = 0u;
             uint32_t v_il_a2 = 0u, v_il_na2 = 0u, v_il_ca2 = 0u, v_il_b2 = 0u, v_il_nb2 = 0u;
@@ -3317,10 +3348,13 @@
                 if (spec) {
                     uint32_t vz;
                     asm volatile("v_mov_b32 %0, 0" : "=v"(vz));
-                    v_a2s = x.rstart[a2 + vz]; v_na2 = x.rnleaf[a2 + vz]; v_cnt2 = m.rcnt[a2 + vz]; v_cap2 = x.rcap[a2 + vz]; v_nb2 = x.rnleaf[b2 + vz];
+                    const uint4* bk_a2 = reinterpret_cast<const uint4*>(x.book + (size_t)(a2 + vz) * RB_WORDS);
+                    const uint4* bk_b2 = reinterpret_cast<const uint4*>(x.book + (size_t)(b2 + vz) * RB_WORDS);
+                    const uint4 r20 = bk_a2[0], r21 = bk_a2[1], q20 = bk_b2[0], q21 = bk_b2[1];
+                    v_a2s = r20.x; v_na2 = r20.y; v_cnt2 = r20.w; v_cap2 = r20.z; v_nb2 = q20.y;
                     v_leaf2 = make_uint2(m.loff[b2 + vz], m.llen[b2 + vz]);
-                    v_b2s = x.rstart[b2 + vz]; v_rows2 = m.rcnt[b2 + vz];
-                    v_il_a2 = x.istart[a2 + vz]; v_il_na2 = x.ilen[a2 + vz]; v_il_ca2 = x.icap[a2 + vz]; v_il_b2 = x.istart[b2 + vz]; v_il_nb2 = x.ilen[b2 + vz];
+                    v_b2s = q20.x; v_rows2 = q20.w;
+                    v_il_a2 = r21.x; v_il_na2 = r21.y; v_il_ca2 = r21.z; v_il_b2 = q21.x; v_il_nb2 = q21.y;
                 }
             }
             float acc = 0.0f;
@@ -3646,8 +3680,16 @@
                     if (commit) {
                         for (int k = 0; k < 3; ++k) { m.rrec[(size_t)a * 16 + k] = cen[k]; m.rrec[(size_t)a * 16 + 3 + k] = n4[k]; }
                         m.rcnt[a] = cnt;
-                        x.rstart[a] = new_start; x.rnleaf[a] = na + nb; x.rcap[a] = new_cap; if (!in_place) s_pool_end = new_start + new_cap;
-                        x.istart[a] = il_new; x.ilen[a] = nt; x.icap[a] = il_newcap; if (!il_in_place) s_ipool_end = il_new + il_newcap;
+    #ifdef F3DS_MERGE_PROF
+                        const unsigned long long tb0 = __builtin_amdgcn_s_memtime();
+    #endif
+                        uint4* bk = reinterpret_cast<uint4*>(x.book + (size_t)a * RB_WORDS);
+                        bk[0] = make_uint4(new_start, na + nb, new_cap, cnt); bk[1] = make_uint4(il_new, nt, il_newcap, 0u);
+    #ifdef F3DS_MERGE_PROF
+                        if (tid == 0) tph_book += __builtin_amdgcn_s_memtime() - tb0;
+    #endif
+                        if (!in_place) s_pool_end = new_start + new_cap;
+                        if (!il_in_place) s_ipool_end = il_new + il_newcap;
                         s_cold.ralive[b] = 0; s_cold.parent[b] = a;
                     }
                 }
@@ -3736,7 +3778,7 @@
 #ifdef F3DS_EXP_DUP_W
                     { const float w0 = quad ? edge_weight_quad(mp, r1, r2, lane & 3, &err, mc) : a_edge_weight(mp, r1, r2, &err, mc); r1[9] += (w0 - w0); }
 #endif
-                    const float w = quad ? edge_weight_quad(mp, r1, r2, lane & 3, &err, mc) : a_edge_weight(mp, r1, r2, &err, mc);
+                    const float w = merge_weight(mp, r1, r2, quad, lane & 3, &err, mc);
                     ku = n_weight_key(w);
                     if (lead && !second) atomicMin(&s_min1, ku);
                 }
@@ -3772,7 +3814,7 @@
 #ifdef F3DS_EXP_DUP_W
                     { const float w0 = quad ? edge_weight_quad(mp, r1, r2, lane & 3, &err, mc) : a_edge_weight(mp, r1, r2, &err, mc); r1[9] += (w0 - w0); }
 #endif
-                    const float w = quad ? edge_weight_quad(mp, r1, r2, lane & 3, &err, mc) : a_edge_weight(mp, r1, r2, &err, mc);
+                    const float w = merge_weight(mp, r1, r2, quad, lane & 3, &err, mc);
                     if (lead) {
                         if (err) { s_cold.dc->error = err; s_err = 1; }
                         publish_edge(e, lo, hi, hprev, n_weight_key(w), epoch, kold);
@@ -3788,12 +3830,14 @@
                         if (tid == 128) {
                             for (int k = 0; k < 12; ++k) m.rrec[(size_t)a2 * 16 + k] = s_rec2[k];
                             m.rcnt[a2] = cnt_a2 + rows2;
-                            x.rstart[a2] = new_start2; x.rnleaf[a2] = na2 + nb2; x.rcap[a2] = new_cap2; if (!in_place2) s_pool_end = new_start2 + new_cap2;
+                            uint4* bk2 = reinterpret_cast<uint4*>(x.book + (size_t)a2 * RB_WORDS);
+                            bk2[0] = make_uint4(new_start2, na2 + nb2, new_cap2, cnt_a2 + rows2); bk2[1] = make_uint4(il_new2, nt2, il_newcap2, 0u);
+                            if (!in_place2) s_pool_end = new_start2 + new_cap2;
                             s_cold.ralive[b2] = 0; s_cold.parent[b2] = a2;
                             const uint32_t wb2 = (kmin2 & 0x80000000u) ? (kmin2 & 0x7fffffffu) : ~kmin2;
                             uint32_t* mg = s_cold.merges; mg[nmerges * 3u] = a2; mg[nmerges * 3u + 1u] = b2; mg[nmerges * 3u + 2u] = wb2;
                             akey[best2] = KEY_DEAD; eab[best2] = 0xFFFFFFFFu; mark_dirty(best2);
-                            x.istart[a2] = il_new2; x.ilen[a2] = nt2; x.icap[a2] = il_newcap2; if (!il_in_place2) s_ipool_end = il_new2 + il_newcap2;
+                            if (!il_in_place2) s_ipool_end = il_new2 + il_newcap2;
                         }
                         for (uint32_t i = tid; i < nt2; i += T) x.ilist[il_new2 + i] = tl2[i];
                         nmerges++; epoch++; sp_hit++;
@@ -3829,10 +3873,10 @@
             const double nm = nmerges ? (double)nmerges : 1.0;
             { const unsigned long long loop_u1 = __builtin_amdgcn_s_memtime(), loop_w1 = __builtin_amdgcn_s_memrealtime();
               printf("  whole loop: %.0f shader clocks, %.1f per tick of the 100 MHz clock (%.2f ms)\n", (double)(loop_u1 - loop_u0), (double)(loop_u1 - loop_u0) / (double)(loop_w1 - loop_w0), (double)(loop_w1 - loop_w0) * 1e-5); }
-            printf("d_merge_il<%d,%d> cycles/merge: argmin (dirty groups + group minima) %.0f [log+meta %.0f list walk %.0f pool %.0f barrier %.0f] [leaves %.0f load+dedupe+store %.0f barrier %.0f fold %.0f] record %.0f weights %.0f  (merges %u, touched/merge %.1f, rows/merge %.1f, tie slow paths %llu)\n",
+            printf("d_merge_il<%d,%d> cycles/merge: argmin (dirty groups + group minima) %.0f [log + book read (two 32-byte records, issued) %.0f list walk %.0f pool %.0f barrier %.0f] [leaves %.0f load+dedupe+store %.0f barrier %.0f fold %.0f] record %.0f weights %.0f  (merges %u, touched/merge %.1f, rows/merge %.1f, tie slow paths %llu)\n",
                    NW, RES, (double)(tph[0] + tph[11] + tph[12] + tph[13] + tph[14] + tph[15]) / nm, (double)tph[5] / nm, (double)tph[6] / nm, (double)tph[7] / nm, (double)tph[1] / nm, (double)tph[8] / nm, (double)tph[9] / nm, (double)tph[10] / nm, (double)tph[2] / nm, (double)tph[3] / nm, (double)tph[4] / nm, nmerges, (double)tph_nt / nm, (double)tph_rows / nm, tph_slow);
             printf("  argmin phase: epoch head %.0f, dirty-group rescan %.0f (%.1f groups per epoch), barrier %.0f, wave 0: group-minima argmin + runner-up %.0f, barrier %.0f, rest %.0f\n", (double)tph[15] / nm, (double)tph[11] / nm, (double)tph_nd / (double)sp_epochs, (double)tph[12] / nm, (double)tph[13] / nm, (double)tph[14] / nm, (double)tph[0] / nm);
-            printf("  record: wave 0 (centroid, normal) %.0f cycles/merge, wave 1 (Lab) %.0f\n", (double)tph_geo / nm, (double)tph_lab / nm);
+            printf("  record: wave 0 (centroid, normal) %.0f cycles/merge, wave 1 (Lab) %.0f, book write-back (issue) %.0f\n", (double)tph_geo / nm, (double)tph_lab / nm, (double)tph_book / nm);
             printf("  speculation: %llu epochs for %u merges; runner-up unique and below the threshold %llu, regions disjoint %llu, second merge small enough %llu, no joining edge %llu, committed %llu\n", sp_epochs, nmerges, sp_cand, sp_disjoint, sp_small, sp_scan, sp_ok);
             for (int k = 0; k < 4; ++k) printf("  rows class %d (<32, <256, <1024, more): %llu merges, %llu rows, leaves+load+fold %.0f cycles/merge = %.1f per row, whole merge %.0f\n", k, cls_n[k], cls_rows[k], cls_n[k] ? (double)cls_fold[k] / cls_n[k] : 0.0, cls_rows[k] ? (double)cls_fold[k] / cls_rows[k] : 0.0, cls_n[k] ? (double)cls_all[k] / cls_n[k] : 0.0);
             for (int k = 0; k < 4; ++k) printf("  touched class %d (<=16, <=64, <=256, more): %llu merges, %llu edges, weights %.0f cycles/merge = %.1f per edge, argmin+scan %.0f, whole merge %.0f\n", k, cle_n[k], cle_nt[k], cle_n[k] ? (double)cle_w[k] / cle_n[k] : 0.0, cle_nt[k] ? (double)cle_w[k] / cle_nt[k] : 0.0, cle_n[k] ? (double)cle_scan[k] / cle_n[k] : 0.0, cle_n[k] ? (double)cle_all[k] / cle_n[k] : 0.0);
```

Result: no change. 3687 (-0.8%).
